# ZhengmaoHe/PARC

Hardware: AMD Instinct MI355X
Metric: env-steps/sec (whole node), 4096 envs/GPU humanoid tracker at 1/2/4/8 MI355X (higher is better)
Workload: dtype f32; 1 GPU; 4096 envs/GPU tracker on procgen box heightfields, 64 synthetic clips (BASELINE.json configs[2]); envs_per_gpu=4096, env_steps_per_bench_step=131072, rollout_steps=32, update_epochs=5, minibatch=16384, sim_substeps=4, parallelism=dp1, scaling_rule=per-rank work fixed (T = 32, minibatch = 4 x envs): weak scaling, grad_allreduce=per minibatch (reference cadence)

## Files before the change

include/parc_hip.h:

```cpp
#ifndef PARC_HIP_H
#define PARC_HIP_H

#include <stdint.h>

#ifdef __cplusplus
extern "C" {
#endif

#define PARC_MAX_BODIES 16
#define PARC_MAX_DOFS 64
#define PARC_MAX_TAR_STEPS 6
#define PARC_MAX_KEY_BODIES 8

#define PARC_OK 0
#define PARC_EINVAL (-1)
#define PARC_EUNSUPPORTED (-2)

#define PARC_JOINT_ROOT 0
#define PARC_JOINT_HINGE 1
#define PARC_JOINT_SPHERICAL 2
#define PARC_JOINT_FIXED 3

#define PARC_DONE_NULL 0
#define PARC_DONE_FAIL 1
#define PARC_DONE_SUCC 2
#define PARC_DONE_TIME 3

typedef struct {
    int32_t num_bodies;
    int32_t dof_size;
    int32_t max_depth;
    int32_t parent[PARC_MAX_BODIES];
    int32_t joint_type[PARC_MAX_BODIES];
    int32_t dof_idx[PARC_MAX_BODIES];
    int32_t depth[PARC_MAX_BODIES];
    float local_translation[PARC_MAX_BODIES][3];
    float local_rotation[PARC_MAX_BODIES][4];
    float joint_axis[PARC_MAX_BODIES][3];
} parc_char_model_t;

typedef struct {
    int32_t num_motions, num_bodies, dof_size, row_stride;
    int32_t off_pos, off_contacts, off_root_vel, off_root_ang_vel, off_dof_vel;
    const int32_t *num_frames;
    const int32_t *start_idx;
    const float *length;
    const int32_t *loop_mode;
    const float *pos_delta;
    const float *frames;
} parc_motion_lib_t;

typedef struct {
    const float *hf;
    int32_t dim_x, dim_y;
    float min_x, min_y, dx, dy;
} parc_terrain_t;

typedef struct {
    int32_t num_tar_steps;
    float tar_dt[PARC_MAX_TAR_STEPS];
    int32_t num_key_bodies;
    int32_t key_body_ids[PARC_MAX_KEY_BODIES];
    float joint_err_w[PARC_MAX_BODIES];
    float dof_err_w[PARC_MAX_DOFS];
    float contact_w[PARC_MAX_BODIES];
    float reward_w[5];
    float rel_deepmimic_w;
    float pose_termination_dist[PARC_MAX_BODIES];
    int32_t pose_termination, enable_early_termination, track_root;
    float root_pos_termination_dist, root_rot_termination_angle, termination_height;
    int32_t num_contact_bodies;
    int32_t contact_body_mask[PARC_MAX_BODIES];
    float episode_length, contact_eps, min_obs_h, max_obs_h;
    int32_t num_ray_points;
    int32_t obs_dim;
    float task1_w, task2_w, target_radius;
    float target_future_min, target_future_max;
    int32_t track_root_h, use_contact_info;
    int32_t global_obs;
} parc_track_cfg_t;

typedef struct {
    int32_t num_envs;
    const float *root_state;
    const float *dof_state;
    const float *rigid_body_state;
    const float *contact_forces;
    const float *env_offsets;
    const int64_t *motion_ids;
    const float *motion_time_offsets;
    const float *motion_xy_offset;
    const float *time_buf;
    const float *target_xy;
    float *ref_root_pos, *ref_root_rot, *ref_root_vel, *ref_root_ang_vel;
    float *ref_joint_rot, *ref_dof_vel, *ref_dof_pos;
    float *ref_contacts, *ref_body_pos;
    float *obs;
    float *reward;
    float *reward_terms;
    int32_t *done;
    int32_t *done_kind;
    const int32_t *env_mask;
    const float *init_noise_xy;
    float *next_target_time;
    const float *target_rand;
    float *obs_aux;
    int32_t reward_terms_stride;
} parc_env_buffers_t;

int parc_refresh_ray_obs_hfs(void *stream, int n_envs, const float *ray_xy, int n_points,
                             const float *root_pos_xyz, const float *heading, parc_terrain_t terrain,
                             float min_h, float max_h, float *out, int64_t out_stride);

int parc_refresh_obs_hfs(void *stream, int n_envs, const float *ray_xy, int n_points, const float *root_state,
                         const float *env_offsets, parc_terrain_t terrain, float min_h, float max_h, float *out,
                         int64_t out_stride);

int parc_dof_to_rot(void *stream, parc_char_model_t model, int n, const float *dof, float *joint_rot);
int parc_rot_to_dof(void *stream, parc_char_model_t model, int n, const float *joint_rot, float *dof);
int parc_forward_kinematics(void *stream, parc_char_model_t model, int n, const float *root_pos, const float *root_rot,
                            const float *joint_rot, float *body_pos, float *body_rot);

int parc_pose_chain_forward(void *stream, parc_char_model_t model, int n, const float *root_pos, const float *root_exp, const float *dof,
                            float *root_quat, float *joint_rot, float *body_pos, float *body_rot);
int parc_pose_chain_backward(void *stream, parc_char_model_t model, int n, const float *root_exp, const float *dof,
                             const float *g_root_quat, const float *g_joint_rot, const float *g_body_pos, const float *g_body_rot,
                             float *g_root_pos, float *g_root_exp, float *g_dof);

int parc_body_points_world(void *stream, int n_frames, int num_bodies, int num_points, const float *body_pos, const float *body_rot,
                           const float *local, const int32_t *owner, float *world);
int parc_body_points_world_grad(void *stream, int n_frames, int num_bodies, int num_points, const float *body_rot, const float *local,
                                const int32_t *start, const float *g_world, float *g_body_pos, float *g_body_rot);

int parc_quat_diff_angle(void *stream, int64_t n, const float *q0, const float *q1, float *angle);
int parc_quat_diff_angle_grad(void *stream, int64_t n, const float *q0, const float *q1, const float *g_angle, float *g_q0, float *g_q1);

int parc_temporal_terms(void *stream, int n_frames, int num_bodies, const float *body_pos, const float *rot_err_sq, const float *src_vel,
                        const float *keep, const float *pair_contact, float c, float c2, float jerk_limit, float *partial);
int parc_temporal_terms_grad(void *stream, int n_frames, int num_bodies, const float *body_pos, const float *rot_err_sq, const float *src_vel,
                             const float *keep, const float *pair_contact, float c, float c2, float jerk_limit, const float *cotangents,
                             float *g_body_pos, float *g_rot_err_sq);

int parc_calc_motion_frame(void *stream, parc_motion_lib_t mlib, int n_queries, const int64_t *motion_ids,
                           const float *motion_times, float *root_pos, float *root_rot, float *root_vel,
                           float *root_ang_vel, float *joint_rot, float *dof_vel, float *contacts);

int parc_motion_lib_build(void *stream, parc_char_model_t model, parc_motion_lib_t mlib, int total_frames,
                          const float *frames, const float *contacts, const int32_t *frame_clip, const float *clip_fps,
                          float *rows);

#define PARC_POST_REF 1
#define PARC_POST_OBS 2
#define PARC_POST_REWARD_DONE 4
#define PARC_POST_HF 8
#define PARC_POST_MASKED 16
#define PARC_POST_INIT_CHAR 32
#define PARC_POST_TARGETS 64
#define PARC_POST_PLAN_CLOCK 128
#define PARC_POST_ALL 255
int parc_track_post_step(void *stream, parc_char_model_t model, parc_motion_lib_t mlib, parc_terrain_t terrain,
                         parc_track_cfg_t cfg, parc_env_buffers_t buf, const int64_t *env_ids, int n_sel, int what,
                         const float *ray_xy);

int parc_track_post_step_timed(void *stream, parc_char_model_t model, parc_motion_lib_t mlib, parc_terrain_t terrain,
                               parc_track_cfg_t cfg, parc_env_buffers_t buf, const int64_t *env_ids, int n_sel, int what,
                               const float *ray_xy, void *start_event, void *stop_event);

int parc_assemble_obs(void *stream, int n_envs, const float *obs, int obs_dim, const float *aux, const float *scalar,
                      const int32_t *col_map, float *out, int out_dim, const int64_t *env_ids, int n_sel);

int parc_reset_apply(void *stream, int n_envs, const int32_t *mask, const int64_t *new_motion_ids, const int64_t *new_terrain_ids,
                     const float *new_time_offsets, const float *motion_offsets, int terrains_per_motion, int64_t *motion_ids,
                     int64_t *motion_terrain_ids, float *motion_time_offsets, float *motion_xy_offset, int32_t *timestep_buf,
                     float *time_buf, int32_t *done, float *next_target_time, int64_t *ep_num);

int parc_reset_sample_apply(void *stream, int n_envs, const int32_t *done_flags, int32_t *mask, const float *uniforms, int n_motions,
                            const float *motion_weights, const float *fail_rates, float min_weight, const float *motion_lengths,
                            const float *motion_offsets, int terrains_per_motion, float noise_scale, float *cdf_workspace,
                            int64_t *motion_ids, int64_t *motion_terrain_ids, float *motion_time_offsets, float *motion_xy_offset,
                            int32_t *timestep_buf, float *time_buf, int32_t *done, float *next_target_time, int64_t *ep_num,
                            float *init_noise_xy);

int parc_step_tail(void *stream, parc_char_model_t model, parc_motion_lib_t mlib, parc_env_buffers_t buf, int what, int n_motions,
                   const int32_t *done_kind, float ema_w, float *fail_rates);
int parc_update_fail_rates(void *stream, int n_envs, int n_motions, const int64_t *motion_ids, const int32_t *done_kind,
                           float ema_w, float *fail_rates);

int parc_td_lambda_return(void *stream, int T, int N, const float *reward, const float *next_vals, const int32_t *done,
                          float discount, float td_lambda, float *ret);
int parc_adv_normalize(void *stream, int n, const float *ret, const float *vals, const float *rand_action_mask,
                       float clip, float *norm_adv, float *mean_std_out , double *workspace);

typedef struct {
    float clip_ratio, bound_w, entropy_w, reg_w, critic_w, large_critic_loss;
    int32_t critic_l1;
} parc_ppo_cfg_t;
int parc_ppo_loss(void *stream, int B, int A, const float *mean, const float *logstd, const float *norm_a, const float *old_logp,
                  const float *adv, const float *mask, const float *pred, const float *tar_val, parc_ppo_cfg_t cfg, float *g_mean,
                  float *g_logstd, float *g_pred, float *out, float *workspace);
int parc_ppo_workspace_floats(int B);
int parc_ppo_loss_packed(void *stream, int B, int A, const float *mean, const float *logstd, const float *rec, int rec_stride,
                         const float *pred, parc_ppo_cfg_t cfg, float *g_mean, float *g_logstd, float *g_pred, float *out,
                         float *workspace);

typedef struct {
    const void *src;
    void *dst;
    int32_t row_bytes;
    int32_t convert;
} parc_record_field_t;
int parc_record_step(void *stream, int n_envs, const int64_t *head, int n_fields, const parc_record_field_t *fields);

int parc_rng_step(void *stream, uint64_t seed, uint64_t *state, float *uniform_out, int64_t n_uniform, float *normal_out, int64_t n_normal,
                  int64_t *tick_cell, int tick_mod);

int64_t parc_sgd_workspace_floats(void);
int parc_sgd_momentum_step(void *stream, int64_t n, float *params, const float *grad, float *momentum_buf, float max_norm, float lr,
                           float momentum, float weight_decay, float *workspace, float *norm_out);

int parc_adamw_step(void *stream, int64_t n, float *params, const float *grad, float *exp_avg, float *exp_avg_sq, int64_t step,
                    float max_norm, float lr, float beta1, float beta2, float eps, float weight_decay, float *workspace, float *norm_out);

int parc_normalize_clamp(void *stream, int64_t rows, int dim, const float *x, const float *mean, const float *stdv, float clip, float *out);

int64_t parc_moments_workspace_floats(int64_t rows, int dim);
int parc_moments_accumulate(void *stream, int64_t rows, int dim, const float *x, float *acc, float *workspace);
int parc_obs_ingest(void *stream, int64_t rows, int dim, const float *x, const float *mean, const float *stdv, float clip, float *norm_out,
                    float *copy_dst, const int64_t *copy_row, float *acc, float *workspace);

int parc_action_head(void *stream, int n, int A, const float *mean, const float *logstd, const float *noise, const float *explore,
                     const float *a_mean, const float *a_std, float *action, float *logp);
int parc_action_head_record(void *stream, int n, int A, const float *mean, const float *logstd, const float *noise, const float *explore,
                            const float *a_mean, const float *a_std, float *action, float *logp, float *rec_action, float *rec_logp,
                            float *rec_mask, const float *forces_src, float *rec_forces, int n_forces, const int64_t *head);

int parc_points_hf_sdf(void *stream, int batch, int n_points, int dim_x, int dim_y, const float *points, const float *hf,
                       const float *min_box_center, const float *x_points, const float *y_points, float half_x, float half_y,
                       float base_z, int inverted, float radius, float *out, int32_t *out_cell);

int parc_points_hf_sdf_grad(void *stream, int batch, int n_points, int dim_x, int dim_y, const float *points, const float *hf,
                            const float *min_box_center, const float *x_points, const float *y_points, float half_x, float half_y,
                            float base_z, int inverted, const int32_t *cell, const float *g_out, float *g_points);

int64_t parc_relu_bwd_workspace_floats(int64_t rows, int dim);
int parc_relu_bwd_bias_grad(void *stream, int64_t rows, int dim, float *gy, const float *y, float *db, float *workspace);
int parc_weighted_colsum(void *stream, int64_t rows, int dim, const float *x, const float *w, float *out, float *workspace);

int parc_abi_version(void);

#ifdef __cplusplus
}
#endif
#endif
```

parc_amd/_hip.py:

```python
import ctypes
import os
import subprocess

import torch

_HERE = os.path.dirname(os.path.abspath(__file__))
LIB_DIR = os.path.join(_HERE, "lib")
LIB_PATH = os.path.join(LIB_DIR, "libparc_hip.so")
CSRC = os.path.join(_HERE, "csrc")
SOURCES = ["parc_kin.hip", "parc_sim.hip", "parc_ppo.hip", "parc_rollout.hip", "parc_optim.hip", "parc_colreduce.hip", "parc_terrain.hip", "parc_render.hip", "parc_score.hip", "parc_netstats.hip", "parc_moopt.hip",
           "parc_augment.hip", "parc_mdm_batch.hip", "parc_mdm_loss.hip", "parc_mdm_guide.hip", "parc_mdm_gen.hip", "parc_hfgather.hip", "parc_motion.hip", "parc_pose_opt.hip", "parc_returns.hip"]
DIAG_LIB_PATH = os.path.join(LIB_DIR, "libparc_hip_diag.so")
DIAG_SOURCES = SOURCES + ["parc_sim_ref.hip"]

MAX_BODIES = 16
MAX_DOFS = 64
MAX_TAR_STEPS = 6
MAX_KEY_BODIES = 8

POST_REF = 1
POST_OBS = 2
POST_REWARD_DONE = 4
POST_HF = 8
POST_MASKED = 16
POST_INIT_CHAR = 32
POST_TARGETS = 64
POST_PLAN_CLOCK = 128

c_int = ctypes.c_int
c_i32 = ctypes.c_int32
c_i64 = ctypes.c_int64
c_f = ctypes.c_float
c_vp = ctypes.c_void_p


class CharModelS(ctypes.Structure):
    _fields_ = [("num_bodies", c_i32), ("dof_size", c_i32), ("max_depth", c_i32),
                ("parent", c_i32 * MAX_BODIES), ("joint_type", c_i32 * MAX_BODIES), ("dof_idx", c_i32 * MAX_BODIES),
                ("depth", c_i32 * MAX_BODIES),
                ("local_translation", (c_f * 3) * MAX_BODIES), ("local_rotation", (c_f * 4) * MAX_BODIES),
                ("joint_axis", (c_f * 3) * MAX_BODIES)]


class MotionLibS(ctypes.Structure):
    _fields_ = [("num_motions", c_i32), ("num_bodies", c_i32), ("dof_size", c_i32), ("row_stride", c_i32),
                ("off_pos", c_i32), ("off_contacts", c_i32), ("off_root_vel", c_i32), ("off_root_ang_vel", c_i32),
                ("off_dof_vel", c_i32),
                ("num_frames", c_vp), ("start_idx", c_vp), ("length", c_vp), ("loop_mode", c_vp), ("pos_delta", c_vp),
                ("frames", c_vp)]


class TerrainS(ctypes.Structure):
    _fields_ = [("hf", c_vp), ("dim_x", c_i32), ("dim_y", c_i32), ("min_x", c_f), ("min_y", c_f), ("dx", c_f), ("dy", c_f)]


class TrackCfgS(ctypes.Structure):
    _fields_ = [("num_tar_steps", c_i32), ("tar_dt", c_f * MAX_TAR_STEPS),
                ("num_key_bodies", c_i32), ("key_body_ids", c_i32 * MAX_KEY_BODIES),
                ("joint_err_w", c_f * MAX_BODIES), ("dof_err_w", c_f * MAX_DOFS), ("contact_w", c_f * MAX_BODIES),
                ("reward_w", c_f * 5), ("rel_deepmimic_w", c_f),
                ("pose_termination_dist", c_f * MAX_BODIES),
                ("pose_termination", c_i32), ("enable_early_termination", c_i32), ("track_root", c_i32),
                ("root_pos_termination_dist", c_f), ("root_rot_termination_angle", c_f), ("termination_height", c_f),
                ("num_contact_bodies", c_i32), ("contact_body_mask", c_i32 * MAX_BODIES),
                ("episode_length", c_f), ("contact_eps", c_f), ("min_obs_h", c_f), ("max_obs_h", c_f),
                ("num_ray_points", c_i32), ("obs_dim", c_i32),
                ("task1_w", c_f), ("task2_w", c_f), ("target_radius", c_f),
                ("target_future_min", c_f), ("target_future_max", c_f), ("track_root_h", c_i32), ("use_contact_info", c_i32), ("global_obs", c_i32)]


class EnvBuffersS(ctypes.Structure):
    _fields_ = [("num_envs", c_i32),
                ("root_state", c_vp), ("dof_state", c_vp), ("rigid_body_state", c_vp), ("contact_forces", c_vp),
                ("env_offsets", c_vp), ("motion_ids", c_vp), ("motion_time_offsets", c_vp), ("motion_xy_offset", c_vp),
                ("time_buf", c_vp), ("target_xy", c_vp),
                ("ref_root_pos", c_vp), ("ref_root_rot", c_vp), ("ref_root_vel", c_vp), ("ref_root_ang_vel", c_vp),
                ("ref_joint_rot", c_vp), ("ref_dof_vel", c_vp), ("ref_dof_pos", c_vp),
                ("ref_contacts", c_vp), ("ref_body_pos", c_vp),
                ("obs", c_vp), ("reward", c_vp), ("reward_terms", c_vp), ("done", c_vp), ("done_kind", c_vp),
                ("env_mask", c_vp), ("init_noise_xy", c_vp), ("next_target_time", c_vp), ("target_rand", c_vp), ("obs_aux", c_vp),
                ("reward_terms_stride", c_i32)]


class RecordFieldS(ctypes.Structure):
    _fields_ = [("src", c_vp), ("dst", c_vp), ("row_bytes", c_i32), ("convert", c_i32)]


class PPOCfgS(ctypes.Structure):
    _fields_ = [("clip_ratio", c_f), ("bound_w", c_f), ("entropy_w", c_f), ("reg_w", c_f), ("critic_w", c_f),
                ("large_critic_loss", c_f), ("critic_l1", c_i32)]


_lib = None


NO_SLP = "-O3 -fno-slp-vectorize"
OPT_LEVEL = {"parc_kin.hip": os.environ.get("PARC_KIN_OPT", NO_SLP), "parc_sim.hip": os.environ.get("PARC_SIM_OPT", NO_SLP), "parc_sim_ref.hip": "-O2",
             "parc_hfgather.hip": NO_SLP, "parc_motion.hip": NO_SLP, "parc_pose_opt.hip": NO_SLP, "parc_returns.hip": NO_SLP,
             "parc_augment.hip": "-O3 -ffp-contract=off",
             "parc_mdm_batch.hip": "-O3 -ffp-contract=off",
             "parc_mdm_loss.hip": "-O3 -ffp-contract=off",
             "parc_mdm_guide.hip": "-O3 -ffp-contract=off",
             "parc_mdm_gen.hip": "-O3 -ffp-contract=off"}


DIGEST_PATH = os.path.join(LIB_DIR, "libparc_hip.digest")
DIAG_DIGEST_PATH = os.path.join(LIB_DIR, "libparc_hip_diag.digest")


def source_digest():
    import hashlib
    h = hashlib.sha256()
    inc = os.path.join(os.path.dirname(_HERE), "include")
    files = [os.path.join(CSRC, f) for f in sorted(os.listdir(CSRC)) if f.endswith((".hip", ".h"))] + \
        ([os.path.join(inc, f) for f in sorted(os.listdir(inc)) if f.endswith(".h")] if os.path.isdir(inc) else [])
    for f in files:
        h.update(os.path.basename(f).encode())
        with open(f, "rb") as fh:
            h.update(fh.read())
    h.update(repr((DIAG_SOURCES, sorted(OPT_LEVEL.items()))).encode())
    return h.hexdigest()


def _stored_digest(path=DIGEST_PATH):
    try:
        with open(path) as f:
            return f.read().strip()
    except OSError:
        return None


def build(force=False, verbose=False, diag=False):
    lib_path, digest_path, sources = (DIAG_LIB_PATH, DIAG_DIGEST_PATH, DIAG_SOURCES) if diag else (LIB_PATH, DIGEST_PATH, SOURCES)
    digest = source_digest()
    if not force and os.path.exists(lib_path) and _stored_digest(digest_path) == digest:
        return lib_path
    obj_dir = os.path.join(LIB_DIR, "obj_diag" if diag else "obj")
    os.makedirs(obj_dir, exist_ok=True)
    hipcc = os.environ.get("HIPCC", "/opt/rocm/bin/hipcc")
    objs, procs = [], []
    for s in sources:
        o = os.path.join(obj_dir, s.replace(".hip", ".o"))
        cmd = [hipcc, "--offload-arch=gfx950"] + OPT_LEVEL.get(s, "-O3").split() + (["-DPARC_DIAG_BUILD"] if diag else []) + \
            ["-std=c++17", "-fPIC", "-c", "-o", o, os.path.join(CSRC, s)]
        if verbose:
            print(" ".join(cmd))
        procs.append((cmd, subprocess.Popen(cmd)))
        objs.append(o)
    for cmd, p in procs:
        if p.wait() != 0:
            raise subprocess.CalledProcessError(p.returncode, cmd)
    cmd = [hipcc, "--offload-arch=gfx950", "-shared", "-fPIC", "-o", lib_path] + objs
    if verbose:
        print(" ".join(cmd))
    subprocess.check_call(cmd)
    with open(digest_path, "w") as f:
        f.write(digest + "\n")
    return lib_path


def lib():
    global _lib
    if _lib is None:
        if not os.path.exists(LIB_PATH):
            raise RuntimeError("libparc_hip.so is not built ({}); run `python -c 'import __graft_entry__ as g; g.build()'` "
                               "-- there is no CPU fallback".format(LIB_PATH))
        if _stored_digest() != source_digest():
            raise RuntimeError("libparc_hip.so was built from other sources than the ones beside it (csrc/, include/): rebuild with "
                               "`python -c 'import __graft_entry__ as g; g.build()'` - calling a stale library would hand it argument "
                               "structs of another layout")
        _lib = ctypes.CDLL(LIB_PATH)
        _declare(_lib)
    return _lib


def _declare(L):
    L.parc_abi_version.restype = c_int
    L.parc_refresh_ray_obs_hfs.argtypes = [c_vp, c_int, c_vp, c_int, c_vp, c_vp, TerrainS, c_f, c_f, c_vp, c_i64]
    L.parc_refresh_obs_hfs.argtypes = [c_vp, c_int, c_vp, c_int, c_vp, c_vp, TerrainS, c_f, c_f, c_vp, c_i64]
    L.parc_dof_to_rot.argtypes = [c_vp, CharModelS, c_int, c_vp, c_vp]
    L.parc_rot_to_dof.argtypes = [c_vp, CharModelS, c_int, c_vp, c_vp]
    L.parc_forward_kinematics.argtypes = [c_vp, CharModelS, c_int, c_vp, c_vp, c_vp, c_vp, c_vp]
    L.parc_pose_chain_forward.argtypes = [c_vp, CharModelS, c_int, c_vp, c_vp, c_vp, c_vp, c_vp, c_vp, c_vp]
    L.parc_pose_chain_backward.argtypes = [c_vp, CharModelS, c_int, c_vp, c_vp, c_vp, c_vp, c_vp, c_vp, c_vp, c_vp, c_vp]
    L.parc_body_points_world.argtypes = [c_vp, c_int, c_int, c_int, c_vp, c_vp, c_vp, c_vp, c_vp]
    L.parc_body_points_world_grad.argtypes = [c_vp, c_int, c_int, c_int, c_vp, c_vp, c_vp, c_vp, c_vp, c_vp]
    L.parc_quat_diff_angle.argtypes = [c_vp, ctypes.c_int64, c_vp, c_vp, c_vp]
    L.parc_quat_diff_angle_grad.argtypes = [c_vp, ctypes.c_int64, c_vp, c_vp, c_vp, c_vp, c_vp]
    L.parc_temporal_terms.argtypes = [c_vp, c_int, c_int, c_vp, c_vp, c_vp, c_vp, c_vp, c_f, c_f, c_f, c_vp]
    L.parc_temporal_terms_grad.argtypes = [c_vp, c_int, c_int, c_vp, c_vp, c_vp, c_vp, c_vp, c_f, c_f, c_f, c_vp, c_vp, c_vp]
    L.parc_calc_motion_frame.argtypes = [c_vp, MotionLibS, c_int, c_vp, c_vp] + [c_vp] * 7
    L.parc_motion_lib_build.argtypes = [c_vp, CharModelS, MotionLibS, c_int, c_vp, c_vp, c_vp, c_vp, c_vp]
    L.parc_track_post_step.argtypes = [c_vp, CharModelS, MotionLibS, TerrainS, TrackCfgS, EnvBuffersS, c_vp, c_int, c_int, c_vp]
    L.parc_track_post_step_timed.argtypes = L.parc_track_post_step.argtypes + [c_vp, c_vp]
    L.parc_track_post_step_timed.restype = c_int
    L.parc_assemble_obs.argtypes = [c_vp, c_int, c_vp, c_int, c_vp, c_vp, c_vp, c_vp, c_int, c_vp, c_int]
    L.parc_assemble_obs.restype = c_int
    L.parc_update_fail_rates.argtypes = [c_vp, c_int, c_int, c_vp, c_vp, c_f, c_vp]
    L.parc_step_tail.argtypes = [c_vp, CharModelS, MotionLibS, EnvBuffersS, c_int, c_int, c_vp, c_f, c_vp]
    L.parc_step_tail.restype = c_int
    L.parc_td_lambda_return.argtypes = [c_vp, c_int, c_int, c_vp, c_vp, c_vp, c_f, c_f, c_vp]
    L.parc_adv_normalize.argtypes = [c_vp, c_int, c_vp, c_vp, c_vp, c_f, c_vp, c_vp, c_vp]
    L.parc_ppo_loss.argtypes = [c_vp, c_int, c_int] + [c_vp] * 8 + [PPOCfgS] + [c_vp] * 5
    L.parc_ppo_loss.restype = c_int
    L.parc_ppo_loss_packed.argtypes = [c_vp, c_int, c_int, c_vp, c_vp, c_vp, c_int, c_vp, PPOCfgS] + [c_vp] * 5
    L.parc_ppo_loss_packed.restype = c_int
    L.parc_ppo_workspace_floats.argtypes = [c_int]
    L.parc_ppo_workspace_floats.restype = c_int
    L.parc_normalize_clamp.argtypes = [c_vp, c_i64, c_int, c_vp, c_vp, c_vp, c_f, c_vp]
    L.parc_normalize_clamp.restype = c_int
    L.parc_action_head.argtypes = [c_vp, c_int, c_int] + [c_vp] * 8
    L.parc_action_head.restype = c_int
    L.parc_action_head_record.argtypes = [c_vp, c_int, c_int] + [c_vp] * 8 + [c_vp] * 5 + [c_int, c_vp]
    L.parc_action_head_record.restype = c_int
    L.parc_points_hf_sdf.argtypes = [c_vp, c_int, c_int, c_int, c_int] + [c_vp] * 5 + [c_f, c_f, c_f, c_int, c_f, c_vp, c_vp]
    L.parc_points_hf_sdf.restype = c_int
    L.parc_points_hf_sdf_grad.argtypes = [c_vp, c_int, c_int, c_int, c_int] + [c_vp] * 5 + [c_f, c_f, c_f, c_int, c_vp, c_vp, c_vp]
    L.parc_points_hf_sdf_grad.restype = c_int
    L.parc_scale_by_clipped_norm.argtypes = [c_vp, c_i64, c_vp, c_vp, c_f]
    L.parc_scale_by_clipped_norm.restype = c_int
    L.parc_moments_workspace_floats.argtypes = [c_i64, c_int]
    L.parc_moments_workspace_floats.restype = c_i64
    L.parc_moments_accumulate.argtypes = [c_vp, c_i64, c_int, c_vp, c_vp, c_vp]
    L.parc_moments_accumulate.restype = c_int
    L.parc_relu_bwd_workspace_floats.argtypes = [c_i64, c_int]
    L.parc_relu_bwd_workspace_floats.restype = c_i64
    L.parc_relu_bwd_bias_grad.argtypes = [c_vp, c_i64, c_int, c_vp, c_vp, c_vp, c_vp]
    L.parc_relu_bwd_bias_grad.restype = c_int
    L.parc_weighted_colsum.argtypes = [c_vp, c_i64, c_int, c_vp, c_vp, c_vp, c_vp]
    L.parc_weighted_colsum.restype = c_int
    L.parc_sgd_workspace_floats.argtypes = []
    L.parc_sgd_workspace_floats.restype = c_i64
    L.parc_sgd_momentum_step.argtypes = [c_vp, c_i64, c_vp, c_vp, c_vp, c_f, c_f, c_f, c_f, c_vp, c_vp]
    L.parc_sgd_momentum_step.restype = c_int
    L.parc_adamw_step.argtypes = [c_vp, c_i64, c_vp, c_vp, c_vp, c_vp, c_i64, c_f, c_f, c_f, c_f, c_f, c_f, c_vp, c_vp]
    L.parc_adamw_step.restype = c_int
    L.parc_return_tracker_update.argtypes = [c_vp, c_int, c_int, c_vp, c_i64] + [c_vp] * 8
    L.parc_return_tracker_workspace_floats.argtypes = [c_int]
    L.parc_return_tracker_workspace_floats.restype = c_i64
    L.parc_return_tracker_update.restype = c_int
    L.parc_record_step.argtypes = [c_vp, c_int, c_vp, c_int, c_vp]
    L.parc_record_step.restype = c_int
    L.parc_obs_ingest.argtypes = [c_vp, c_i64, c_int, c_vp, c_vp, c_vp, c_f, c_vp, c_vp, c_vp, c_vp, c_vp]
    L.parc_obs_ingest.restype = c_int
    L.parc_rng_step.argtypes = [c_vp, ctypes.c_uint64, c_vp, c_vp, c_i64, c_vp, c_i64, c_vp, c_int]
    L.parc_rng_step.restype = c_int
    L.parc_reset_apply.argtypes = [c_vp, c_int, c_vp, c_vp, c_vp, c_vp, c_vp, c_int] + [c_vp] * 9
    L.parc_reset_apply.restype = c_int
    L.parc_reset_sample_apply.argtypes = [c_vp, c_int, c_vp, c_vp, c_vp, c_int, c_vp, c_vp, c_f, c_vp, c_vp, c_int, c_f] + [c_vp] * 11
    L.parc_reset_sample_apply.restype = c_int
    for name in ("parc_refresh_ray_obs_hfs", "parc_refresh_obs_hfs", "parc_dof_to_rot", "parc_rot_to_dof",
                 "parc_forward_kinematics", "parc_calc_motion_frame", "parc_motion_lib_build", "parc_track_post_step", "parc_reset_apply",
                 "parc_update_fail_rates", "parc_td_lambda_return", "parc_adv_normalize"):
        getattr(L, name).restype = c_int
    if hasattr(L, "parc_sim_abi"):
        from . import _hip_sim
        _hip_sim.declare(L)
    if hasattr(L, "parc_render_abi"):
        from . import _hip_render
        _hip_render.declare(L)
    if hasattr(L, "parc_score_abi"):
        from . import _hip_score
        _hip_score.declare(L)
    if hasattr(L, "parc_netstats_abi"):
        from . import _hip_netstats
        _hip_netstats.declare(L)
    if hasattr(L, "parc_moopt_abi"):
        from . import _hip_moopt
        _hip_moopt.declare(L)
    if hasattr(L, "parc_augment_abi"):
        from . import _hip_augment
        _hip_augment.declare(L)
    if hasattr(L, "parc_mdm_batch_abi"):
        from . import _hip_mdm_batch
        _hip_mdm_batch.declare(L)
    if hasattr(L, "parc_mdm_loss_abi"):
        from . import _hip_mdm_loss
        _hip_mdm_loss.declare(L)
    if hasattr(L, "parc_mdm_guide_abi"):
        from . import _hip_mdm_guide
        _hip_mdm_guide.declare(L)
    if hasattr(L, "parc_mdm_gen_abi"):
        from . import _hip_mdm_gen
        _hip_mdm_gen.declare(L)


EXPORTED = ["parc_abi_version", "parc_refresh_ray_obs_hfs", "parc_refresh_obs_hfs", "parc_dof_to_rot", "parc_rot_to_dof",
            "parc_forward_kinematics", "parc_calc_motion_frame", "parc_motion_lib_build", "parc_track_post_step",
            "parc_update_fail_rates", "parc_td_lambda_return", "parc_adv_normalize", "parc_reset_apply", "parc_ppo_loss", "parc_ppo_workspace_floats", "parc_record_step", "parc_return_tracker_update", "parc_normalize_clamp",
            "parc_action_head", "parc_points_hf_sdf", "parc_moments_workspace_floats", "parc_moments_accumulate", "parc_reset_sample_apply", "parc_return_tracker_workspace_floats", "parc_scale_by_clipped_norm", "parc_relu_bwd_workspace_floats",
            "parc_relu_bwd_bias_grad", "parc_ppo_loss_packed", "parc_weighted_colsum", "parc_sgd_workspace_floats", "parc_sgd_momentum_step", "parc_adamw_step",
            "parc_pose_chain_forward", "parc_pose_chain_backward", "parc_points_hf_sdf_grad", "parc_body_points_world", "parc_body_points_world_grad",
            "parc_quat_diff_angle", "parc_quat_diff_angle_grad", "parc_temporal_terms", "parc_temporal_terms_grad", "parc_step_tail",
            "parc_assemble_obs", "parc_track_post_step_timed", "parc_rng_step", "parc_obs_ingest", "parc_action_head_record",
            "parc_render", "parc_render_abi", "parc_motion_score", "parc_score_abi",
            "parc_netstats_workspace_floats", "parc_netstats_update", "parc_netstats_abs_colsum", "parc_netstats_dormant_count", "parc_netstats_abi",
            "parc_points_hf_sdf_ragged", "parc_points_hf_sdf_ragged_grad", "parc_temporal_terms_seg", "parc_temporal_terms_seg_grad",
            "parc_segment_sums", "parc_moopt_abi",
            "parc_augment_frames", "parc_augment_terrains", "parc_augment_localize", "parc_augment_abi",
            "parc_mdm_heightfields", "parc_mdm_windows", "parc_mdm_batch_abi",
            "parc_mdm_loss_forward", "parc_mdm_loss_backward", "parc_mdm_loss_lds_bytes", "parc_mdm_loss_abi",
            "parc_mdm_guide_step", "parc_mdm_guide_lds_bytes", "parc_mdm_guide_abi",
            "parc_mdm_gen_encode", "parc_mdm_gen_decode", "parc_mdm_gen_abi"]


def check(rc, what):
    if rc != 0:
        raise RuntimeError("{} failed with code {} ({})".format(what, rc, "bad argument" if rc == -1 else "unsupported" if rc == -2 else "hipError"))


def stream():
    return c_vp(torch.cuda.current_stream().cuda_stream)


def ptr(t):
    if t is None:
        return c_vp(0)
    assert t.is_cuda, "HIP kernels need device tensors (no CPU fallback)"
    assert t.is_contiguous(), "tensor must be contiguous"
    return c_vp(t.data_ptr())


def terrain_struct(hf, min_point, dxdy):
    assert hf.dtype == torch.float32 and hf.is_contiguous() and hf.dim() == 2
    return TerrainS(ptr(hf), int(hf.shape[0]), int(hf.shape[1]), float(min_point[0]), float(min_point[1]),
                    float(dxdy[0]), float(dxdy[1]))


class HipEventPair:
    _rt = None

    def __init__(self):
        if HipEventPair._rt is None:
            HipEventPair._rt = ctypes.CDLL("libamdhip64.so")
        self.start, self.stop = c_vp(), c_vp()
        for ev in (self.start, self.stop):
            rc = HipEventPair._rt.hipEventCreate(ctypes.byref(ev))
            if rc != 0:
                raise RuntimeError("hipEventCreate -> %d" % rc)

    def elapsed_us(self):
        ms = ctypes.c_float()
        rc = HipEventPair._rt.hipEventElapsedTime(ctypes.byref(ms), self.start, self.stop)
        if rc != 0:
            raise RuntimeError("hipEventElapsedTime -> %d" % rc)
        return ms.value * 1e3

    def __del__(self):
        try:
            for ev in (self.start, self.stop):
                if ev:
                    HipEventPair._rt.hipEventDestroy(ev)
        except Exception:
            pass
```

parc_amd/csrc/parc_colreduce.hip:

```cpp
#include <hip/hip_runtime.h>
#include <stdint.h>

#include "../../include/parc_hip.h"
#include "parc_launch.h"
#include "parc_learner_math.h"

__global__ __launch_bounds__(256) void normalize_clamp_kernel(size_t n4, int dim4, const float4 *__restrict__ x, const float4 *__restrict__ mean,
                                                              const float4 *__restrict__ stdv, float clip, float4 *__restrict__ out) {
    for (size_t i = (size_t)blockIdx.x * blockDim.x + threadIdx.x; i < n4; i += (size_t)gridDim.x * blockDim.x) {
        const int c = (int)(i % (size_t)dim4);
        const float4 v = x[i], m = mean[c], s = stdv[c];
        float4 o;
        o.x = clamp_nan((v.x - m.x) / s.x, -clip, clip);
        o.y = clamp_nan((v.y - m.y) / s.y, -clip, clip);
        o.z = clamp_nan((v.z - m.z) / s.z, -clip, clip);
        o.w = clamp_nan((v.w - m.w) / s.w, -clip, clip);
        out[i] = o;
    }
}

extern "C" int parc_normalize_clamp(void *stream, int64_t rows, int dim, const float *x, const float *mean, const float *stdv, float clip,
                                    float *out) {
    if (rows < 0 || dim <= 0 || (dim & 3) || (((uintptr_t)x | (uintptr_t)mean | (uintptr_t)stdv | (uintptr_t)out) & 15)) return PARC_EINVAL;
    if (rows == 0) return PARC_OK;
    const size_t n4 = (size_t)rows * (size_t)(dim / 4);
    hipLaunchKernelGGL(normalize_clamp_kernel, dim3(parc_capped_blocks(n4, 8192)), dim3(256), 0, (hipStream_t)stream, n4, dim / 4, (const float4 *)x,
                       (const float4 *)mean, (const float4 *)stdv, clip, (float4 *)out);
    PARC_CHECK_LAUNCH();
    return PARC_OK;
}

struct col_chunk_t {
    int lane, rg, c, r0, r1;
};

__device__ __forceinline__ col_chunk_t col_chunk(int rows, int chunk_rows) {
    const int lane = threadIdx.x & 63, r0 = blockIdx.y * chunk_rows;
    return {lane, (int)(threadIdx.x >> 6), (int)(blockIdx.x * 64 + lane), r0, min(r0 + chunk_rows, rows)};
}

__device__ __forceinline__ float4 fold_row_groups(const float4 (*red)[64], int lane) {
    const float4 a = red[0][lane], b = red[1][lane], d = red[2][lane], e = red[3][lane];
    float4 o;
    o.x = (a.x + b.x) + (d.x + e.x); o.y = (a.y + b.y) + (d.y + e.y); o.z = (a.z + b.z) + (d.z + e.z); o.w = (a.w + b.w) + (d.w + e.w);
    return o;
}

__device__ __forceinline__ void fold_store(float4 (*red)[64], const float4 &s, const col_chunk_t &k, int dim4, float4 *__restrict__ partial) {
    red[k.rg][k.lane] = s;
    __syncthreads();
    if (k.rg == 0 && k.c < dim4) partial[(size_t)blockIdx.y * dim4 + k.c] = fold_row_groups(red, k.lane);
}

__device__ __forceinline__ void fold_store_moments(float4 (*red)[4][64], const float4 &s, const float4 &q, const col_chunk_t &k, int dim4,
                                                   float4 *__restrict__ partial) {
    red[0][k.rg][k.lane] = s;
    red[1][k.rg][k.lane] = q;
    __syncthreads();
    if (k.rg < 2 && k.c < dim4) partial[((size_t)blockIdx.y * 2 + k.rg) * dim4 + k.c] = fold_row_groups(red[k.rg], k.lane);
}

struct col_grid_t {
    int rc, dim4, chunks;
    dim3 grid;
};

static col_grid_t col_chunk_grid(int64_t rows, int dim, int chunk_rows, uintptr_t aligned16, bool missing) {
    if (rows < 0 || dim <= 0 || (dim & 3) || missing || (aligned16 & 15)) return {PARC_EINVAL};
    if (rows > (int64_t)chunk_rows * 65535) return {PARC_EUNSUPPORTED};
    const int dim4 = dim / 4, chunks = (int)((rows + chunk_rows - 1) / chunk_rows);
    return {PARC_OK, dim4, chunks, dim3((dim4 + 63) / 64, chunks)};
}

#define MOM_ROWS 64
__global__ __launch_bounds__(256) void moments_partial_kernel(int rows, int dim4, const float4 *__restrict__ x, float4 *__restrict__ partial) {
    __shared__ float4 red[2][4][64];
    const col_chunk_t k = col_chunk(rows, MOM_ROWS);
    const int rg = k.rg, c = k.c, r0 = k.r0, r1 = k.r1;
    float4 s = make_float4(0.f, 0.f, 0.f, 0.f), q = s;
    if (c < dim4) {
        for (int r = r0 + rg; r < r1; r += 4) {
            const float4 v = x[(size_t)r * dim4 + c];
            s.x += v.x; s.y += v.y; s.z += v.z; s.w += v.w;
            q.x = fmaf(v.x, v.x, q.x); q.y = fmaf(v.y, v.y, q.y); q.z = fmaf(v.z, v.z, q.z); q.w = fmaf(v.w, v.w, q.w);
        }
    }
    fold_store_moments(red, s, q, k, dim4, partial);
}

__global__ __launch_bounds__(256) void obs_ingest_kernel(int rows, int dim4, const float4 *__restrict__ x, const float4 *__restrict__ mean,
                                                         const float4 *__restrict__ stdv, float clip, float4 *__restrict__ norm_out,
                                                         float4 *copy_dst, const int64_t *__restrict__ copy_row, float4 *partial) {
    __shared__ float4 red[2][4][64];
    const col_chunk_t k = col_chunk(rows, MOM_ROWS);
    const int rg = k.rg, c = k.c, r0 = k.r0, r1 = k.r1;
    float4 s = make_float4(0.f, 0.f, 0.f, 0.f), q = s;
    if (c < dim4) {
        const float4 m = mean[c], sd = stdv[c];
        float4 *dst = copy_dst ? copy_dst + (size_t)copy_row[0] * (size_t)rows * dim4 : nullptr;
        for (int r = r0 + rg; r < r1; r += 4) {
            const size_t i = (size_t)r * dim4 + c;
            const float4 v = x[i];
            float4 o;
            o.x = clamp_nan((v.x - m.x) / sd.x, -clip, clip);
            o.y = clamp_nan((v.y - m.y) / sd.y, -clip, clip);
            o.z = clamp_nan((v.z - m.z) / sd.z, -clip, clip);
            o.w = clamp_nan((v.w - m.w) / sd.w, -clip, clip);
            norm_out[i] = o;
            if (dst) {
                typedef float f32x4 __attribute__((ext_vector_type(4)));
                f32x4 vv = {v.x, v.y, v.z, v.w};
                __builtin_nontemporal_store(vv, reinterpret_cast<f32x4 *>(dst) + i);
            }
            s.x += v.x; s.y += v.y; s.z += v.z; s.w += v.w;
            q.x = fmaf(v.x, v.x, q.x); q.y = fmaf(v.y, v.y, q.y); q.z = fmaf(v.z, v.z, q.z); q.w = fmaf(v.w, v.w, q.w);
        }
    }
    if (!partial) return;
    fold_store_moments(red, s, q, k, dim4, partial);
}

__global__ __launch_bounds__(256) void moments_final_kernel(int chunks, int dim4, const float4 *__restrict__ partial, float4 *acc) {
    const int i = blockIdx.x * blockDim.x + threadIdx.x;
    if (i >= 2 * dim4) return;
    const int which = i / dim4, c = i - which * dim4;
    float4 t = make_float4(0.f, 0.f, 0.f, 0.f);
#pragma unroll 16
    for (int k = 0; k < chunks; ++k) {
        const float4 v = partial[((size_t)k * 2 + which) * dim4 + c];
        t.x += v.x; t.y += v.y; t.z += v.z; t.w += v.w;
    }
    float4 a = acc[i];
    a.x += t.x; a.y += t.y; a.z += t.z; a.w += t.w;
    acc[i] = a;
}

static void launch_moments_final(void *stream, const col_grid_t &g, const float *workspace, float *acc) {
    hipLaunchKernelGGL(moments_final_kernel, dim3((2 * g.dim4 + 255) / 256), dim3(256), 0, (hipStream_t)stream, g.chunks, g.dim4,
                       (const float4 *)workspace, (float4 *)acc);
}

extern "C" int64_t parc_moments_workspace_floats(int64_t rows, int dim) {
    if (rows < 0 || dim <= 0) return -1;
    return ((rows + MOM_ROWS - 1) / MOM_ROWS) * 2 * (int64_t)dim;
}

extern "C" int parc_obs_ingest(void *stream, int64_t rows, int dim, const float *x, const float *mean, const float *stdv, float clip, float *norm_out,
                               float *copy_dst, const int64_t *copy_row, float *acc, float *workspace) {
    const col_grid_t g = col_chunk_grid(rows, dim, MOM_ROWS,
                                        (uintptr_t)x | (uintptr_t)mean | (uintptr_t)stdv | (uintptr_t)norm_out | (uintptr_t)copy_dst | (uintptr_t)acc | (uintptr_t)workspace,
                                        !x || !mean || !stdv || !norm_out || (copy_dst && !copy_row) || (acc && !workspace));
    if (g.rc != PARC_OK || rows == 0) return g.rc;
    hipLaunchKernelGGL(obs_ingest_kernel, g.grid, dim3(256), 0, (hipStream_t)stream, (int)rows, g.dim4, (const float4 *)x, (const float4 *)mean,
                       (const float4 *)stdv, clip, (float4 *)norm_out, (float4 *)copy_dst, copy_row, acc ? (float4 *)workspace : (float4 *)nullptr);
    if (acc) launch_moments_final(stream, g, workspace, acc);
    PARC_CHECK_LAUNCH();
    return PARC_OK;
}

extern "C" int parc_moments_accumulate(void *stream, int64_t rows, int dim, const float *x, float *acc, float *workspace) {
    const col_grid_t g = col_chunk_grid(rows, dim, MOM_ROWS, (uintptr_t)x | (uintptr_t)acc | (uintptr_t)workspace, false);
    if (g.rc != PARC_OK || rows == 0) return g.rc;
    hipLaunchKernelGGL(moments_partial_kernel, g.grid, dim3(256), 0, (hipStream_t)stream, (int)rows, g.dim4, (const float4 *)x, (float4 *)workspace);
    launch_moments_final(stream, g, workspace, acc);
    PARC_CHECK_LAUNCH();
    return PARC_OK;
}

#define RB_ROWS 128
__global__ __launch_bounds__(256) void relu_bwd_bias_partial_kernel(int rows, int dim4, float4 *__restrict__ gy, const float4 *__restrict__ y,
                                                                    float4 *__restrict__ partial) {
    __shared__ float4 red[4][64];
    const col_chunk_t k = col_chunk(rows, RB_ROWS);
    const int rg = k.rg, c = k.c, r0 = k.r0, r1 = k.r1;
    float4 s = make_float4(0.f, 0.f, 0.f, 0.f);
    if (c < dim4) {
#pragma unroll 4
        for (int r = r0 + rg; r < r1; r += 4) {
            const size_t i = (size_t)r * dim4 + c;
            float4 g = gy[i];
            const float4 a = y[i];
            g.x = a.x <= 0.f ? 0.f : g.x; g.y = a.y <= 0.f ? 0.f : g.y; g.z = a.z <= 0.f ? 0.f : g.z; g.w = a.w <= 0.f ? 0.f : g.w;
            gy[i] = g;
            s.x += g.x; s.y += g.y; s.z += g.z; s.w += g.w;
        }
    }
    fold_store(red, s, k, dim4, partial);
}

__global__ __launch_bounds__(256) void colsum_final_kernel(int chunks, int dim, const float *__restrict__ partial, float *__restrict__ out) {
    const int c = blockIdx.x * blockDim.x + threadIdx.x;
    if (c >= dim) return;
    float t = 0.f;
#pragma unroll 16
    for (int k = 0; k < chunks; ++k) t += partial[(size_t)k * dim + c];
    out[c] = t;
}

__global__ __launch_bounds__(256) void weighted_colsum_partial_kernel(int rows, int dim4, const float4 *__restrict__ x, const float *__restrict__ w,
                                                                      float4 *__restrict__ partial) {
    __shared__ float4 red[4][64];
    const col_chunk_t k = col_chunk(rows, RB_ROWS);
    const int rg = k.rg, c = k.c, r0 = k.r0, r1 = k.r1;
    float4 s = make_float4(0.f, 0.f, 0.f, 0.f);
    if (c < dim4) {
#pragma unroll 4
        for (int r = r0 + rg; r < r1; r += 4) {
            const float4 v = x[(size_t)r * dim4 + c];
            const float wr = w[r];
            s.x = fmaf(wr, v.x, s.x); s.y = fmaf(wr, v.y, s.y); s.z = fmaf(wr, v.z, s.z); s.w = fmaf(wr, v.w, s.w);
        }
    }
    fold_store(red, s, k, dim4, partial);
}

static void launch_colsum_final(void *stream, const col_grid_t &g, int dim, const float *workspace, float *out) {
    hipLaunchKernelGGL(colsum_final_kernel, dim3((dim + 255) / 256), dim3(256), 0, (hipStream_t)stream, g.chunks, dim, workspace, out);
}

extern "C" int parc_weighted_colsum(void *stream, int64_t rows, int dim, const float *x, const float *w, float *out, float *workspace) {
    const col_grid_t g = col_chunk_grid(rows, dim, RB_ROWS, (uintptr_t)x | (uintptr_t)workspace, !x || !w || !out || !workspace);
    if (g.rc != PARC_OK) return g.rc;
    if (rows > 0)
        hipLaunchKernelGGL(weighted_colsum_partial_kernel, g.grid, dim3(256), 0, (hipStream_t)stream, (int)rows, g.dim4, (const float4 *)x, w,
                           (float4 *)workspace);
    launch_colsum_final(stream, g, dim, workspace, out);
    PARC_CHECK_LAUNCH();
    return PARC_OK;
}

extern "C" int64_t parc_relu_bwd_workspace_floats(int64_t rows, int dim) {
    if (rows < 0 || dim <= 0) return -1;
    return ((rows + RB_ROWS - 1) / RB_ROWS) * (int64_t)dim;
}

extern "C" int parc_relu_bwd_bias_grad(void *stream, int64_t rows, int dim, float *gy, const float *y, float *db, float *workspace) {
    const col_grid_t g = col_chunk_grid(rows, dim, RB_ROWS, (uintptr_t)gy | (uintptr_t)y | (uintptr_t)workspace, !gy || !y || !db || !workspace);
    if (g.rc != PARC_OK) return g.rc;
    if (rows > 0)
        hipLaunchKernelGGL(relu_bwd_bias_partial_kernel, g.grid, dim3(256), 0, (hipStream_t)stream, (int)rows, g.dim4, (float4 *)gy, (const float4 *)y,
                           (float4 *)workspace);
    launch_colsum_final(stream, g, dim, workspace, db);
    PARC_CHECK_LAUNCH();
    return PARC_OK;
}
```

parc_amd/csrc/parc_ppo.hip:

```cpp
#include <hip/hip_runtime.h>

#include "../../include/parc_hip.h"
#include "parc_launch.h"
#include "parc_learner_math.h"

#define PPO_THREADS 256
#define PPO_MAX_A 64
#define PPO_NSCAL 8
#define PPO_W (PPO_NSCAL + PPO_MAX_A)

struct ppo_surr_t {
    float ratio, surr, c;
};

__device__ __forceinline__ ppo_surr_t ppo_surrogate(int A, float zz, float sum_logstd, const float *old_logp, const float *adv, size_t si, bool sel,
                                                    float m, parc_ppo_cfg_t cfg) {
    ppo_surr_t s;
    const float logp = -0.5f * zz + (-0.5f * (float)A * 1.8378770664093453f - sum_logstd);
    s.ratio = __expf(logp - old_logp[si]);
    const float ad = adv[si];
    const float lo = 1.0f - cfg.clip_ratio, hi = 1.0f + cfg.clip_ratio;
    const float rc = clamp_nan(s.ratio, lo, hi);
    const float l0 = ad * s.ratio, l1 = ad * rc;
    s.surr = minimum_nan(l0, l1);
    const float dsurr = (l0 <= l1) ? ad : ((s.ratio >= lo && s.ratio <= hi) ? ad : 0.f);
    s.c = sel ? -m * dsurr * s.ratio : 0.f;
    return s;
}

__device__ __forceinline__ float ppo_critic_grad(parc_ppo_cfg_t cfg, float diff) {
    return cfg.critic_l1 ? (diff > 0.f ? -1.f : (diff < 0.f ? 1.f : 0.f)) : -2.0f * diff;
}

__global__ __launch_bounds__(PPO_THREADS) void ppo_sample_kernel(int B, int A, const float *__restrict__ mean, const float *__restrict__ logstd,
                                                                 const float *__restrict__ norm_a, const float *__restrict__ old_logp,
                                                                 const float *__restrict__ adv, const float *__restrict__ mask,
                                                                 const float *__restrict__ pred, const float *__restrict__ tar_val,
                                                                 parc_ppo_cfg_t cfg, float *g_mean, float *g_pred, float *ws, int a_stride,
                                                                 int s_stride) {
    __shared__ float s_istd[PPO_MAX_A];
    __shared__ float s_part[PPO_THREADS / 64][PPO_W];
    const int tid = threadIdx.x, i = blockIdx.x * PPO_THREADS + tid;
    float sum_logstd = 0.f;
    if (tid < A) s_istd[tid] = __expf(-logstd[tid]);
    __syncthreads();
    for (int j = 0; j < A; ++j) sum_logstd += logstd[j];
    const bool live = i < B;
    const int ii = live ? i : 0;
    const size_t si = (size_t)ii * s_stride;
    const bool sel = live && mask[si] == 1.0f;
    const float m = sel ? 1.f : 0.f;
    const float *mu = mean + (size_t)ii * A, *ac = norm_a + (size_t)ii * a_stride;
    float zz = 0.f, viol = 0.f, reg = 0.f;
    for (int j = 0; j < A; ++j) {
        float mj = mu[j];
        float z = (ac[j] - mj) * s_istd[j];
        zz = fmaf(z, z, zz);
        float vmin = clamp_max_nan(mj + 1.0f, 0.f), vmax = clamp_min_nan(mj - 1.0f, 0.f);
        viol += vmin * vmin + vmax * vmax;
        reg = fmaf(mj, mj, reg);
    }
    const ppo_surr_t sr = ppo_surrogate(A, zz, sum_logstd, old_logp, adv, si, sel, m, cfg);
    const float c = sr.c;
    const float diff = tar_val[si] - pred[ii];
    if (live) {
        g_pred[i] = ppo_critic_grad(cfg, diff);
        float *gm = g_mean + (size_t)i * A;
        for (int j = 0; j < A; ++j) {
            float mj = mu[j];
            float z = (ac[j] - mj) * s_istd[j];
            float vmin = clamp_max_nan(mj + 1.0f, 0.f), vmax = clamp_min_nan(mj - 1.0f, 0.f);
            gm[j] = sel ? c * z * s_istd[j] + m * (cfg.bound_w * 2.0f * (vmin + vmax) + cfg.reg_w * 2.0f * mj) : 0.f;
        }
    }
    float sc[PPO_NSCAL];
    sc[0] = m;
    sc[1] = live ? (cfg.critic_l1 ? fabsf(diff) : diff * diff) : 0.f;
    sc[2] = sel ? m * sr.surr : 0.f;
    sc[3] = m * (fabsf(sr.ratio - 1.0f) > cfg.clip_ratio ? 1.f : 0.f);
    sc[4] = sel ? m * sr.ratio : 0.f;
    sc[5] = sel ? m * viol : 0.f;
    sc[6] = sel ? m * reg : 0.f;
    sc[7] = 0.f;
    const int wv = tid >> 6, ln = tid & 63;
#pragma unroll
    for (int k = 0; k < PPO_NSCAL; ++k) {
        float v = wave_sum(sc[k]);
        if (ln == 0) s_part[wv][k] = v;
    }
    for (int j = 0; j < A; ++j) {
        float z = live ? (ac[j] - mu[j]) * s_istd[j] : 0.f;
        float v = wave_sum(sel ? c * (z * z - 1.0f) : 0.f);
        if (ln == 0) s_part[wv][PPO_NSCAL + j] = v;
    }
    __syncthreads();
    if (tid < PPO_NSCAL + A) {
        float v = 0.f;
#pragma unroll
        for (int w = 0; w < PPO_THREADS / 64; ++w) v += s_part[w][tid];
        ws[(size_t)blockIdx.x * PPO_W + tid] = v;
    }
}

#define PPO32_SPB 64
__global__ __launch_bounds__(256) void ppo_sample32_kernel(int B, int A, const float *__restrict__ mean, const float *__restrict__ logstd,
                                                           const float *__restrict__ norm_a, const float *__restrict__ old_logp,
                                                           const float *__restrict__ adv, const float *__restrict__ mask,
                                                           const float *__restrict__ pred, const float *__restrict__ tar_val, parc_ppo_cfg_t cfg,
                                                           float *g_mean, float *g_pred, float *ws, int a_stride, int s_stride) {
    __shared__ float s_part[8][PPO_W];
    const int tid = threadIdx.x, g = tid >> 5, j = tid & 31;
    const bool vj = j < A;
    const float ls = vj ? logstd[j] : 0.f;
    const float istd = __expf(-ls);
    float sum_logstd = ls;
#pragma unroll
    for (int o = 16; o >= 1; o >>= 1) sum_logstd += __shfl_xor(sum_logstd, o, 32);
    float acc[PPO_NSCAL];
#pragma unroll
    for (int k = 0; k < PPO_NSCAL; ++k) acc[k] = 0.f;
    float acc_ls = 0.f;
#pragma unroll 2
    for (int it = 0; it < PPO32_SPB / 8; ++it) {
        const int i = blockIdx.x * PPO32_SPB + it * 8 + g;
        const bool live = i < B;
        const int ii = live ? i : 0;
        const size_t si = (size_t)ii * s_stride;
        const bool sel = live && mask[si] == 1.0f;
        const float m = sel ? 1.f : 0.f;
        const float mj = vj ? mean[(size_t)ii * A + j] : 0.f;
        const float aj = vj ? norm_a[(size_t)ii * a_stride + j] : 0.f;
        const float z = (aj - mj) * istd;
        const float vmin = clamp_max_nan(mj + 1.0f, 0.f), vmax = clamp_min_nan(mj - 1.0f, 0.f);
        float zz = vj ? z * z : 0.f, viol = vj ? vmin * vmin + vmax * vmax : 0.f, reg = vj ? mj * mj : 0.f;
#pragma unroll
        for (int o = 16; o >= 1; o >>= 1) {
            zz += __shfl_xor(zz, o, 32);
            viol += __shfl_xor(viol, o, 32);
            reg += __shfl_xor(reg, o, 32);
        }
        const ppo_surr_t sr = ppo_surrogate(A, zz, sum_logstd, old_logp, adv, si, sel, m, cfg);
        const float c = sr.c;
        const float diff = tar_val[si] - pred[ii];
        if (live) {
            if (j == 0) g_pred[i] = ppo_critic_grad(cfg, diff);
            if (vj) g_mean[(size_t)i * A + j] = sel ? c * z * istd + m * (cfg.bound_w * 2.0f * (vmin + vmax) + cfg.reg_w * 2.0f * mj) : 0.f;
        }
        acc[0] += m;
        acc[1] += live ? (cfg.critic_l1 ? fabsf(diff) : diff * diff) : 0.f;
        acc[2] += sel ? m * sr.surr : 0.f;
        acc[3] += m * (fabsf(sr.ratio - 1.0f) > cfg.clip_ratio ? 1.f : 0.f);
        acc[4] += sel ? m * sr.ratio : 0.f;
        acc[5] += sel ? m * viol : 0.f;
        acc[6] += sel ? m * reg : 0.f;
        acc_ls += (sel && vj) ? c * (z * z - 1.0f) : 0.f;
    }
    if (j == 0) {
#pragma unroll
        for (int k = 0; k < PPO_NSCAL; ++k) s_part[g][k] = acc[k];
    }
    if (vj) s_part[g][PPO_NSCAL + j] = acc_ls;
    __syncthreads();
    if (tid < PPO_NSCAL + A) {
        float v = 0.f;
#pragma unroll
        for (int w = 0; w < 8; ++w) v += s_part[w][tid];
        ws[(size_t)blockIdx.x * PPO_W + tid] = v;
    }
}

#define PPO_RED_THREADS (4 * PPO_W)
__global__ __launch_bounds__(PPO_RED_THREADS) void ppo_reduce_kernel(int B, int A, int nblk, const float *__restrict__ logstd, parc_ppo_cfg_t cfg,
                                                                    const float *__restrict__ ws, float *g_logstd, float *out) {
    __shared__ float s[PPO_W];
    __shared__ double s4[PPO_W][4];
    const int tid = threadIdx.x;
    {
        const int v = tid >> 2, part = tid & 3;
        const int per = (nblk + 3) >> 2, b0 = part * per, b1 = min(b0 + per, nblk);
        double acc = 0.0;
        if (v < PPO_NSCAL + A) {
#pragma unroll 16
            for (int b = b0; b < b1; ++b) acc += (double)ws[(size_t)b * PPO_W + v];
        }
        s4[v][part] = acc;
    }
    __syncthreads();
    if (tid < PPO_NSCAL + A) s[tid] = (float)((s4[tid][0] + s4[tid][1]) + (s4[tid][2] + s4[tid][3]));
    __syncthreads();
    const float msum = s[0];
    const float cnt = msum;
    const float critic_loss = s[1] / (float)B;
    float sum_logstd = 0.f;
    for (int j = 0; j < A; ++j) sum_logstd += logstd[j];
    const float ent = (sum_logstd + 0.5f * (float)A * 2.8378770664093453f) * (msum / cnt);
    const float abl = s[5] / cnt, regl = s[6] / cnt;
    float actor_loss = -s[2] / cnt;
    if (cfg.bound_w != 0.f) actor_loss += cfg.bound_w * abl;
    if (cfg.entropy_w != 0.f) actor_loss -= cfg.entropy_w * ent;
    if (cfg.reg_w != 0.f) actor_loss += cfg.reg_w * regl;
    const float gate = critic_loss > cfg.large_critic_loss ? 0.f : 1.f;
    if (tid < A) g_logstd[tid] = gate * (s[PPO_NSCAL + tid] / cnt - cfg.entropy_w * (msum / cnt));
    if (tid == 0) {
        out[0] = actor_loss + cfg.critic_w * critic_loss;
        out[1] = critic_loss;
        out[2] = actor_loss;
        out[3] = s[3] / cnt;
        out[4] = s[4] / cnt;
        out[5] = abl;
        out[6] = ent;
        out[7] = regl;
        out[8] = cnt;
        out[9] = gate / cnt;
        out[10] = cfg.critic_w / (float)B;
    }
}

__global__ __launch_bounds__(256) void ppo_scale_kernel(int n_mean, int n_pred, const float *__restrict__ out, float *g_mean, float *g_pred) {
    const int i = blockIdx.x * blockDim.x + threadIdx.x;
    const float sa = out[9], sp = out[10];
    if (i < n_mean) g_mean[i] *= sa;
    if (i < n_pred) g_pred[i] *= sp;
}

static int ppo_loss_impl(void *stream, int B, int A, const float *mean, const float *logstd, const float *norm_a, const float *old_logp,
                         const float *adv, const float *mask, const float *pred, const float *tar_val, parc_ppo_cfg_t cfg, float *g_mean,
                         float *g_logstd, float *g_pred, float *out, float *workspace, int a_stride, int s_stride) {
    if (B <= 0 || A <= 0 || A > PPO_MAX_A) return PARC_EINVAL;
    int nblk = (B + PPO_THREADS - 1) / PPO_THREADS;
    hipStream_t st = (hipStream_t)stream;
    if (A <= 32) {
        nblk = (B + PPO32_SPB - 1) / PPO32_SPB;
        hipLaunchKernelGGL(ppo_sample32_kernel, dim3(nblk), dim3(256), 0, st, B, A, mean, logstd, norm_a, old_logp, adv, mask, pred, tar_val, cfg,
                           g_mean, g_pred, workspace, a_stride, s_stride);
    } else {
        hipLaunchKernelGGL(ppo_sample_kernel, dim3(nblk), dim3(PPO_THREADS), 0, st, B, A, mean, logstd, norm_a, old_logp, adv, mask, pred, tar_val,
                           cfg, g_mean, g_pred, workspace, a_stride, s_stride);
    }
    hipLaunchKernelGGL(ppo_reduce_kernel, dim3(1), dim3(PPO_RED_THREADS), 0, st, B, A, nblk, logstd, cfg, workspace, g_logstd, out);
    const int n = B * A;
    hipLaunchKernelGGL(ppo_scale_kernel, dim3((n + 255) / 256), dim3(256), 0, st, n, B, out, g_mean, g_pred);
    PARC_CHECK_LAUNCH();
    return PARC_OK;
}

extern "C" int parc_ppo_loss(void *stream, int B, int A, const float *mean, const float *logstd, const float *norm_a, const float *old_logp,
                             const float *adv, const float *mask, const float *pred, const float *tar_val, parc_ppo_cfg_t cfg, float *g_mean,
                             float *g_logstd, float *g_pred, float *out, float *workspace) {
    return ppo_loss_impl(stream, B, A, mean, logstd, norm_a, old_logp, adv, mask, pred, tar_val, cfg, g_mean, g_logstd, g_pred, out, workspace, A, 1);
}

extern "C" int parc_ppo_loss_packed(void *stream, int B, int A, const float *mean, const float *logstd, const float *rec, int rec_stride,
                                    const float *pred, parc_ppo_cfg_t cfg, float *g_mean, float *g_logstd, float *g_pred, float *out,
                                    float *workspace) {
    if (!rec || rec_stride < A + 4) return PARC_EINVAL;
    return ppo_loss_impl(stream, B, A, mean, logstd, rec, rec + A, rec + A + 1, rec + A + 2, pred, rec + A + 3, cfg, g_mean, g_logstd, g_pred, out,
                         workspace, rec_stride, rec_stride);
}

extern "C" int parc_ppo_workspace_floats(int B) { return ((B + PPO32_SPB - 1) / PPO32_SPB) * PPO_W; }
```

parc_amd/learning/dm_ppo_agent.py:

```python
import enum
import os
import time

import numpy as np
import torch

from ..envs import base_env
from ..gym_spaces import Box
from ..util import mp_util
from ..util.logger import Logger
from . import dm_ppo_model, experience_buffer, mp_optimizer, normalizer, rl_util, unit_stats
from .dm_ppo_return_tracker import DMPPOReturnTracker
from .tracking_error_tracker import TrackingErrorTracker


class AgentMode(enum.Enum):
    TRAIN = 0
    TEST = 1


_LOSS_KEYS = ["norm_obs", "action", "a_logp", "tar_val", "adv", "rand_action_mask"]


def enable_tuned_gemms():
    import torch.cuda.tunable as tunable
    path = os.path.join(os.path.dirname(os.path.dirname(os.path.abspath(__file__))), "tunableop_results.csv")
    if not os.path.exists(path) or tunable.is_enabled():
        return
    tunable.set_filename(path, False)
    tunable.tuning_enable(False)
    if hasattr(tunable, "write_file_on_exit"):
        tunable.write_file_on_exit(False)
    tunable.enable(True)


class DMPPOAgent(torch.nn.Module):
    NAME = "DM_PPO"

    def __init__(self, config, env, device):
        super().__init__()
        self._env = env
        self._device = device
        self._iter = 0
        self._sample_count = 0
        self._config = config
        self._is_terrain_runner = env.NAME in ("ig_terrain_runner", "ig_parkour")
        self._has_target_task = env.NAME in ("ig_terrain_runner", "ig_deepmimic_terrain", "ig_parkour")
        self._load_params(config)
        self._build_normalizers()
        self._model = dm_ppo_model.DMPPOModel(config["model"], env)
        self.to(self._device)
        params = [p for p in self.parameters() if p.requires_grad]
        self._optimizer = mp_optimizer.MPOptimizer(config["optimizer"], params)
        self._build_exp_buffer(config)
        self._train_return_tracker = DMPPOReturnTracker(self.get_num_envs(), self._device, self._has_target_task)
        self._test_return_tracker = DMPPOReturnTracker(self.get_num_envs(), self._device, self._has_target_task)
        self._mode = AgentMode.TRAIN
        self._curr_obs = None
        self._curr_info = None
        self._ppo_cfg = None
        if str(self._device).startswith("cuda") and config.get("tuned_gemms", True):
            enable_tuned_gemms()
        self._use_hip_graph = bool(config.get("hip_graph_rollout", True)) and str(self._device).startswith("cuda")
        self._graphs = dict()
        self._graph_pool = None
        self._graph_warm = 0
        self._exp_prob_t = torch.ones([1, 1], dtype=torch.float32, device=self._device)
        self._head_t = torch.zeros([1], dtype=torch.int64, device=self._device)
        self._head_dev, self._exp_prob_dev = 0, 1.0
        self._compute_times = []
        self._replan_time_rows, self._replan_time_src = None, None
        self._ones_mask = None
        self._unit_stats = None
        self._unit_report = None
        if getattr(self._env, "_report_tracking_error", False):
            self._test_tracking_error_tracker = TrackingErrorTracker(self.get_num_envs(), self._device)

    @staticmethod
    def rollout_shape(config, num_procs):
        P = int(num_procs) if config.get("mp_scale_rollout", True) else 1
        return int(np.ceil(config["steps_per_iter"] / P)), int(np.ceil(config["batch_size"] / P))

    def _load_params(self, config):
        self._discount = config["discount"]
        self._iters_per_output = config["iters_per_output"]
        self._iters_per_checkpoint = config["iters_per_checkpoint"]
        self._normalizer_samples = config.get("normalizer_samples", np.inf)
        self._test_episodes = config["test_episodes"]
        self._steps_per_iter, self._batch_size = self.rollout_shape(config, mp_util.get_num_procs())
        self._update_epochs = config["update_epochs"]
        self._td_lambda = config["td_lambda"]
        self._ppo_clip_ratio = config["ppo_clip_ratio"]
        self._norm_adv_clip = config["norm_adv_clip"]
        self._action_bound_weight = config["action_bound_weight"]
        self._action_entropy_weight = config["action_entropy_weight"]
        self._action_reg_weight = config["action_reg_weight"]
        self._critic_loss_weight = config["critic_loss_weight"]
        self._exp_anneal_samples = config.get("exp_anneal_samples", np.inf)
        self._exp_prob_beg = config.get("exp_prob_beg", 1.0)
        self._exp_prob_end = config.get("exp_prob_end", 1.0)
        self._clip_grad_norm = config.get("clip_grad_norm", False)
        self._max_grad_norm = config.get("max_grad_norm", 0.5)
        self._critic_loss_type = config.get("critic_loss_type", "L2")
        self._log_unit_stats = bool(config.get("log_unit_stats", False))

    def _build_normalizers(self):
        obs_space = self._env.get_obs_space()
        shapes = self._env._compute_obs(ret_obs_shapes=True)
        idx, cur = [], 0
        for key in shapes:
            shape = shapes[key]["shape"]
            flat = shape[0] * shape[1] if len(shape) >= 2 else shape[0]
            if not shapes[key]["use_normalizer"]:
                idx.append(torch.arange(cur, cur + flat, dtype=torch.int64, device=self._device))
            cur += flat
        non_norm = torch.cat(idx) if idx else None
        self._obs_norm = normalizer.Normalizer(obs_space.shape, device=self._device, dtype=torch.float32, non_norm_indices=non_norm,
                                               clip=self._config["norm_obs_clip"])
        a_space = self._env.get_action_space()
        assert isinstance(a_space, Box)
        a_mean = torch.tensor(0.5 * (a_space.high + a_space.low), device=self._device, dtype=torch.float32)
        a_std = torch.tensor(0.5 * (a_space.high - a_space.low), device=self._device, dtype=torch.float32)
        self._a_norm = normalizer.Normalizer(a_mean.shape, device=self._device, init_mean=a_mean, init_std=a_std, dtype=torch.float32)

    def _build_exp_buffer(self, config):
        T, N, dev = self._steps_per_iter, self.get_num_envs(), self._device
        self._exp_buffer = experience_buffer.ExperienceBuffer(buffer_length=T, batch_size=N, device=dev)
        obs_dim = list(self._env.get_obs_space().shape)
        a_dim = list(self._env.get_action_space().shape)
        B = self._env._cfg.num_bodies if hasattr(self._env, "_cfg") else 15

        def add(name, shape, dtype=torch.float32):
            self._exp_buffer.add_buffer(name, torch.zeros([T, N] + shape, device=dev, dtype=dtype))
        add("obs", obs_dim)
        add("next_obs", obs_dim)
        add("action", a_dim)
        add("reward", [])
        add("done", [], torch.int)
        add("a_logp", [])
        add("tar_val", [])
        add("adv", [])
        add("rand_action_mask", [])
        add("timestep", [], torch.int)
        add("ep_num", [], torch.int)
        add("compute_time", [])
        add("prev_char_contact_forces", [B, 3])
        add("next_char_contact_forces", [B, 3])
        add("env_id", [], torch.int64)
        add("norm_obs", obs_dim)
        self._loss_rec_w = ((a_dim[0] if isinstance(a_dim, (list, tuple)) else int(a_dim)) + 4 + 3) // 4 * 4
        add("loss_rec", [self._loss_rec_w])
        self._env_ids = torch.arange(0, N, 1, device=dev, dtype=torch.int64)
        if self._is_terrain_runner:
            add("replan_timer", [])
            add("replan_counter", [], torch.int64)

    def get_num_envs(self):
        return self._env.get_num_envs()

    def get_action_size(self):
        return int(np.prod(self._env.get_action_space().shape))

    def calc_num_params(self):
        return sum(p.numel() for p in self.parameters() if p.requires_grad)

    def set_mode(self, mode):
        self._mode = mode
        self._env.set_mode(base_env.EnvMode.TRAIN if mode == AgentMode.TRAIN else base_env.EnvMode.TEST)

    def save(self, out_file):
        if mp_util.is_root_proc():
            torch.save(self.state_dict(), out_file)

    def load(self, in_file):
        self.load_state_dict(torch.load(in_file, map_location=self._device, weights_only=True))
        self._optimizer.sync()
        Logger.print("Loaded model parameters from {:s}".format(in_file))

    def _get_exp_prob(self):
        if np.isfinite(self._exp_anneal_samples):
            l = float(np.clip(float(self._sample_count) / self._exp_anneal_samples, 0.0, 1.0))
            return (1.0 - l) * self._exp_prob_beg + l * self._exp_prob_end
        return self._exp_prob_beg

    def _set_exp_prob(self, exp_prob):
        if not getattr(self, "_in_graph_step", False):
            self._exp_prob_t.fill_(exp_prob)
            self._exp_prob_dev = exp_prob

    def _need_normalizer_update(self):
        return self._sample_count < self._normalizer_samples

    @torch.no_grad()
    def _decide_action(self, obs, info):
        self._obs_ingested = self._action_recorded = False
        if getattr(self, "_in_graph_step", False) and self._mode == AgentMode.TRAIN and self._obs_norm.can_ingest(obs) \
                and obs.shape[0] == self.get_num_envs() and self._exp_buffer._device_head is not None:
            norm_obs = self._obs_norm.ingest(obs, record=self._need_normalizer_update(),
                                             copy_into=(self._exp_buffer.get_data("obs"), self._exp_buffer._device_head))
            self._obs_ingested = True
        else:
            norm_obs = self._obs_norm.normalize(obs)
        dist = self._model.eval_actor(norm_obs) if self._unit_stats is None else self._eval_actor_with_unit_stats(norm_obs)
        if obs.is_cuda and dist.logstd.dim() == 2 and dist.logstd.stride(0) == 0 and self._config.get("fused_action_head", True):
            return self._decide_action_fused(dist, obs.shape[0])
        if self._mode == AgentMode.TRAIN:
            exp_prob = self._get_exp_prob()
            if exp_prob >= 1.0:
                norm_a = dist.sample()
                mask = torch.ones_like(norm_a[..., 0])
            else:
                self._set_exp_prob(exp_prob)
                mask = torch.bernoulli(self._exp_prob_t.expand(obs.shape[0], 1))
                norm_a = torch.where(mask == 1.0, dist.sample(), dist.mode)
                mask = mask.squeeze(-1)
        else:
            norm_a = dist.mode
            mask = torch.zeros_like(norm_a[..., 0])
        logp = dist.log_prob(norm_a)
        a = self._a_norm.unnormalize(norm_a)
        return a, {"a_logp": logp, "rand_action_mask": mask}

    def _decide_action_fused(self, dist, n):
        from .. import _hip
        mean = dist.mean.contiguous()
        A = mean.shape[1]
        if self._mode == AgentMode.TRAIN:
            exp_prob = self._get_exp_prob()
            if exp_prob >= 1.0:
                if self._ones_mask is None or self._ones_mask.shape[0] != n:
                    self._ones_mask = torch.ones(n, dtype=torch.float32, device=mean.device)
                mask = self._ones_mask
            else:
                self._set_exp_prob(exp_prob)
                mask = torch.bernoulli(self._exp_prob_t.expand(n, 1)).squeeze(-1).contiguous()
            noise = self._step_noise if (getattr(self, "_step_noise", None) is not None and self._step_noise.shape == mean.shape) else torch.randn_like(mean)
        else:
            mask = torch.zeros(n, dtype=torch.float32, device=mean.device)
            noise = mean
        a = torch.empty_like(mean)
        logp = torch.empty(n, dtype=torch.float32, device=mean.device)
        p = _hip.ptr
        eb = self._exp_buffer
        self._action_recorded = False
        if (getattr(self, "_in_graph_step", False) and self._mode == AgentMode.TRAIN and A <= 32 and eb._device_head is not None and n == self.get_num_envs()
                and hasattr(self._env, "_char_contact_forces")):
            f = self._env._char_contact_forces
            nf = f[0].numel()
            _hip.check(_hip.lib().parc_action_head_record(_hip.stream(), n, A, p(mean), p(dist.logstd[0].contiguous()), p(noise), p(mask),
                                                          p(self._a_norm.get_mean()), p(self._a_norm.get_std()), p(a), p(logp),
                                                          p(eb.get_data("action")), p(eb.get_data("a_logp")), p(eb.get_data("rand_action_mask")),
                                                          p(f.contiguous()), p(eb.get_data("prev_char_contact_forces")), nf, p(eb._device_head)),
                       "parc_action_head_record")
            self._action_recorded = True
            return a, {"a_logp": logp, "rand_action_mask": mask}
        _hip.check(_hip.lib().parc_action_head(_hip.stream(), n, A, p(mean), p(dist.logstd[0].contiguous()), p(noise), p(mask),
                                               p(self._a_norm.get_mean()), p(self._a_norm.get_std()), p(a), p(logp)), "parc_action_head")
        return a, {"a_logp": logp, "rand_action_mask": mask}

    def _eval_actor_with_unit_stats(self, norm_obs):
        st = self._unit_stats
        dist, acts = self._model.eval_actor_tapped(norm_obs)
        st.update(acts, dist.mean)
        if st.print_every and st.steps % st.print_every == 0:
            Logger.print("\n".join(unit_stats.report_lines(st.report())))
        return dist

    def _unit_stats_on(self, print_every=0):
        self._unit_stats = unit_stats.UnitStats(self._model, self.get_num_envs(), self._device, tap=getattr(self, "_unit_stats_tap", None))
        self._unit_stats.print_every = int(print_every)

    def _unit_stats_off(self, ranks=None):
        st, self._unit_stats = self._unit_stats, None
        if st is not None:
            self._unit_report = dict(st.report())
            if ranks is not None:
                self._unit_report = {"ranks": ranks, **self._unit_report}

    def unit_report(self):
        return self._unit_report

    def test_model2(self, num_episodes, verbose=False, k=100):
        unit_stats.check_model(self._model)
        self.eval()
        self.set_mode(AgentMode.TEST)
        ranks = unit_stats.model_rank_figures(self._model)
        Logger.print("\n".join(unit_stats.rank_lines(ranks)))
        self._curr_obs, self._curr_info = self._env.reset()
        self._unit_stats_on(print_every=k if verbose else 0)
        try:
            info = self._rollout_test(int(np.ceil(num_episodes / mp_util.get_num_procs())))
            self._unit_stats_off(ranks)
        finally:
            self._unit_stats = None
        Logger.print("\n".join(unit_stats.report_lines(self._unit_report)))
        return info

    def step(self):
        action, action_info = self._decide_action(self._curr_obs, self._curr_info)
        next_obs, r, done, next_info = self._env.step(action)
        return next_obs, r, done, next_info, action, action_info

    def _record_data_pre_step(self, obs, info, action, action_info):
        eb = self._exp_buffer
        if getattr(self, "_in_graph_step", False):
            ingested = getattr(self, "_obs_ingested", False)
            if self._need_normalizer_update() and not ingested:
                self._obs_norm.record(obs)
            items = [] if ingested else [("obs", obs)]
            if not getattr(self, "_action_recorded", False):
                items += [("action", action), ("a_logp", action_info["a_logp"]), ("rand_action_mask", action_info["rand_action_mask"]),
                          ("prev_char_contact_forces", self._env._char_contact_forces)]
            if items:
                eb.record_group(items)
            return
        eb.record("obs", obs)
        eb.record("action", action)
        if self._need_normalizer_update():
            self._obs_norm.record(obs)
        eb.record("a_logp", action_info["a_logp"])
        eb.record("rand_action_mask", action_info["rand_action_mask"])
        eb.record("prev_char_contact_forces", self._env._char_contact_forces if getattr(self, "_in_graph_step", False)
                  else info["char_contact_forces"])

    def _record_data_post_step(self, next_obs, r, done, next_info):
        eb = self._exp_buffer
        if getattr(self, "_in_graph_step", False):
            items = [("next_obs", next_obs), ("reward", r), ("done", done), ("timestep", next_info["timestep"]),
                     ("ep_num", next_info["ep_num"]), ("next_char_contact_forces", next_info["char_contact_forces"]),
                     ("env_id", self._env_ids)]
            if self._is_terrain_runner:
                items += [("replan_timer", self._env.get_replan_time_buf()), ("replan_counter", self._env.get_replan_counter())]
            eb.record_group(items)
            return
        eb.record("next_obs", next_obs)
        eb.record("reward", r)
        eb.record("done", done)
        eb.record("timestep", next_info["timestep"])
        eb.record("ep_num", next_info["ep_num"])
        if not getattr(self, "_in_graph_step", False):
            eb.get_data("compute_time")[eb._buffer_head].fill_(float(next_info["compute_time"]))
        eb.record("next_char_contact_forces", next_info["char_contact_forces"])
        eb.record("env_id", self._env_ids)
        if self._is_terrain_runner:
            eb.record("replan_timer", self._env.get_replan_time_buf().expand(self.get_num_envs()))
            eb.record("replan_counter", self._env.get_replan_counter())

    def _reset_done_envs(self, done):
        done_indices = (done != base_env.DoneFlags.NULL.value).nonzero(as_tuple=False).flatten()
        return self._env.reset(done_indices)

    def _device_tick(self):
        return hasattr(self._env, "step_randoms") and self._config.get("device_step_randoms", True)

    def _train_step_body(self, device_reset=False):
        self._step_noise = None
        if getattr(self, "_in_graph_step", False) and self._device_tick():
            self._step_noise = self._env.step_randoms(self.get_action_size(), tick=(self._head_t, self._exp_buffer._buffer_length))
        action, action_info = self._decide_action(self._curr_obs, self._curr_info)
        self._record_data_pre_step(self._curr_obs, self._curr_info, action, action_info)
        next_obs, r, done, next_info = self._env.step(action)
        self._train_return_tracker.update(next_info, done)
        self._record_data_post_step(next_obs, r, done, next_info)
        if device_reset:
            self._curr_obs, self._curr_info = self._env.reset_done(done)
        return done

    def _device_reset_ok(self):
        env = self._env
        return self._graph_ok() and hasattr(env, "reset_done") and env.supports_device_reset()

    def _graph_ok(self):
        env = self._env
        return (self._use_hip_graph and self._mode == AgentMode.TRAIN and not getattr(env, "_write_agent_states_flag", False)
                and hasattr(env, "_char_contact_forces") and getattr(getattr(env, "_core", None), "timing_events", None) is None
                and getattr(env, "supports_graph_step", lambda: True)())

    def _train_step_graph(self, device_reset=False):
        eb = self._exp_buffer
        exp_prob = self._get_exp_prob()
        sig = self._env.host_step_signature() if hasattr(self._env, "host_step_signature") else ()
        key = (self._need_normalizer_update(), exp_prob >= 1.0, device_reset) + tuple(sig)
        want = (eb._buffer_head - 1) % eb._buffer_length if self._device_tick() else eb._buffer_head
        if self._head_dev != want:
            self._head_t.fill_(want)
            self._head_dev = want
        if self._exp_prob_dev != exp_prob:
            self._exp_prob_t.fill_(exp_prob)
            self._exp_prob_dev = exp_prob
        g = self._graphs.get(key)
        if g is None:
            if self._graph_warm < 2:
                self._graph_warm += 1
                return self._train_step_body(device_reset)
            eb.set_device_head(self._head_t)
            self._in_graph_step = True
            snapshots = getattr(self._env, "_info_snapshots", None)
            if snapshots is not None:
                self._env._info_snapshots = False
            count0 = self._obs_norm._new_count
            host0 = self._env.host_step_state() if hasattr(self._env, "host_step_state") else None
            captured = False
            try:
                torch.cuda.synchronize()
                g = torch.cuda.CUDAGraph()
                with torch.cuda.graph(g, pool=self._graph_pool, capture_error_mode="thread_local"):
                    done = self._train_step_body(device_reset)
                if self._graph_pool is None:
                    self._graph_pool = g.pool()
                captured = True
            except Exception as exc:
                Logger.print("hipGraph capture of the rollout step failed ({}); continuing with eager launches".format(exc))
                self._use_hip_graph = False
            finally:
                eb.set_device_head(None)
                self._in_graph_step = False
                if snapshots is not None:
                    self._env._info_snapshots = snapshots
            self._obs_norm._new_count = count0
            if not captured:
                torch.cuda.synchronize()
                if hasattr(self._env, "restore_host_step_state"):
                    self._env.restore_host_step_state(host0)
                done = self._train_step_body(False)
                self._graph_fallback_reset = True
                return done
            self._graphs[key] = (g, done)
            fresh = True
        else:
            fresh = False
        g, done = self._graphs[key]
        g.replay()
        if self._device_tick():
            self._head_dev = (self._head_dev + 1) % eb._buffer_length
        if not fresh and hasattr(self._env, "host_step_replayed"):
            self._env.host_step_replayed()
        if key[0]:
            self._obs_norm._new_count += self.get_num_envs()
        self._compute_times.append((eb._buffer_head, time.time() - self._env._start_compute_time))
        return done

    def _flush_compute_times(self):
        if self._compute_times:
            rows = torch.tensor([r for r, _ in self._compute_times], dtype=torch.long, device=self._device)
            vals = torch.tensor([v for _, v in self._compute_times], dtype=torch.float32, device=self._device)
            buf = self._exp_buffer.get_data("compute_time")
            buf[rows] = vals.unsqueeze(1).expand(-1, buf.shape[1])
            self._compute_times = []

    def _rollout_train(self, num_steps):
        for _ in range(num_steps):
            if self._graph_ok():
                dev_reset = self._device_reset_ok()
                done = self._train_step_graph(dev_reset)
                if getattr(self, "_graph_fallback_reset", False):
                    self._graph_fallback_reset = False
                    dev_reset = False
            else:
                dev_reset = False
                done = self._train_step_body()
            if not dev_reset:
                self._curr_obs, self._curr_info = self._reset_done_envs(done)
            self._exp_buffer.inc()
        self._flush_compute_times()

    def _rollout_test(self, num_episodes):
        self._test_return_tracker.reset()
        report_te = getattr(self._env, "_report_tracking_error", False)
        if report_te:
            self._test_tracking_error_tracker.reset()
        if num_episodes == 0:
            return {"mean_return": 0.0, "mean_ep_len": 0.0, "num_eps": 0}
        min_eps_per_env = int(np.ceil(num_episodes / self.get_num_envs()))
        while True:
            action, _ = self._decide_action(self._curr_obs, self._curr_info)
            _, _, done, next_info = self._env.step(action)
            self._test_return_tracker.update(next_info, done)
            if report_te and "tracking_error" in next_info:
                self._test_tracking_error_tracker.update(next_info["tracking_error"], done)
            self._curr_obs, self._curr_info = self._reset_done_envs(done)
            if torch.all(self._test_return_tracker.get_eps_per_env() > min_eps_per_env - 1):
                break
        out = {"mean_return": self._test_return_tracker.get_mean_return().item(),
               "mean_ep_len": self._test_return_tracker.get_mean_ep_len().item(),
               "num_eps": self._test_return_tracker.get_episodes()}
        if report_te:
            t = self._test_tracking_error_tracker
            out.update({"test_mean_root_pos_tracking_err": t.get_mean_root_pos_err().item(),
                        "test_mean_root_rot_tracking_err": t.get_mean_root_rot_err().item(),
                        "test_mean_body_pos_tracking_err": t.get_mean_body_pos_err().item(),
                        "test_mean_body_rot_tracking_err": t.get_mean_body_rot_err().item(),
                        "test_mean_dof_vel_tracking_err": t.get_mean_dof_vel_err().item(),
                        "test_mean_root_vel_tracking_err": t.get_mean_root_vel_err().item(),
                        "test_mean_root_ang_vel_tracking_err": t.get_mean_root_ang_vel_err().item()})
        return out

    def hard_reset_envs(self):
        if self._is_terrain_runner:
            self._env.apply_hard_reset()
        self._curr_obs, self._curr_info = self._env.reset()

    def test_model(self, num_episodes):
        self.eval()
        self.set_mode(AgentMode.TEST)
        self.hard_reset_envs()
        P = mp_util.get_num_procs()
        return self._rollout_test(int(np.ceil(num_episodes / P)))

    @torch.no_grad()
    def _critic_values(self):
        eb = self._exp_buffer
        obs, next_obs, done = eb.get_data("obs"), eb.get_data("next_obs"), eb.get_data("done")
        norm_obs = self._obs_norm.normalize(obs, out=eb.get_data("norm_obs"))
        vals = self._model.eval_critic(norm_obs).squeeze(-1)
        T = obs.shape[0]
        need = done != base_env.DoneFlags.NULL.value
        need[T - 1] = True
        next_vals = torch.empty_like(vals)
        next_vals[:T - 1] = vals[1:]
        idx = need.flatten().nonzero().flatten()
        sel = next_obs.flatten(0, 1)[idx]
        next_vals.flatten()[idx] = self._model.eval_critic(self._obs_norm.normalize(sel)).squeeze(-1)
        return vals, next_vals

    @torch.no_grad()
    def _build_train_data(self):
        self.eval()
        eb = self._exp_buffer
        obs, next_obs = eb.get_data("obs"), eb.get_data("next_obs")
        r, done = eb.get_data("reward"), eb.get_data("done")
        mask = eb.get_data("rand_action_mask")
        vals, next_vals = self._critic_values()
        r_min, r_max = self._env.get_reward_bounds()
        next_vals = torch.clamp(next_vals, r_min / (1.0 - self._discount), r_max / (1.0 - self._discount))
        succ_val = self._env.get_reward_succ() / (1.0 - self._discount)
        fail_val = self._env.get_reward_fail() / (1.0 - self._discount)
        next_vals = torch.where(done == base_env.DoneFlags.SUCC.value, torch.full_like(next_vals, succ_val), next_vals)
        next_vals = torch.where(done == base_env.DoneFlags.FAIL.value, torch.full_like(next_vals, fail_val), next_vals)
        new_vals = rl_util.compute_td_lambda_return(r, next_vals, done, self._discount, self._td_lambda)
        norm_adv, mean_std = rl_util.normalize_advantage(new_vals, vals, mask, self._norm_adv_clip)
        eb.set_data("tar_val", new_vals)
        eb.set_data("adv", norm_adv)
        if eb.has_buffer("loss_rec"):
            rec = eb.get_data("loss_rec")
            A = eb.get_data("action").shape[-1]
            self._a_norm.normalize(eb.get_data("action"), out=rec[..., 0:A])
            rec[..., A] = eb.get_data("a_logp")
            rec[..., A + 1] = norm_adv
            rec[..., A + 2] = mask
            rec[..., A + 3] = new_vals
        return {"adv_mean": mean_std[0], "adv_std": mean_std[1]}

    def _compute_loss(self, batch):
        norm_obs = batch["norm_obs"] if "norm_obs" in batch else self._obs_norm.normalize(batch["obs"])
        norm_a = self._a_norm.normalize(batch["action"])
        pred = self._model.eval_critic(norm_obs).squeeze(-1)
        if norm_obs.is_cuda and self._config.get("fused_ppo_loss", True):
            fused = self._compute_loss_fused(batch, norm_obs, norm_a, pred)
            if fused is not None:
                return fused
        diff = batch["tar_val"] - pred
        critic_loss = torch.mean(torch.square(diff)) if self._critic_loss_type == "L2" else torch.mean(torch.abs(diff))
        m = (batch["rand_action_mask"] == 1.0).to(torch.float32)
        cnt = m.sum().clamp_min(1.0)
        a_dist = self._model.eval_actor(norm_obs)
        a_logp = a_dist.log_prob(norm_a)
        ratio = torch.exp(a_logp - batch["a_logp"])
        adv = batch["adv"]
        l0 = adv * ratio
        l1 = adv * torch.clamp(ratio, 1.0 - self._ppo_clip_ratio, 1.0 + self._ppo_clip_ratio)
        actor_loss = -(torch.minimum(l0, l1) * m).sum() / cnt
        info = {"critic_loss": critic_loss.detach(), "clip_frac": (((torch.abs(ratio - 1.0) > self._ppo_clip_ratio).float() * m).sum() / cnt).detach(),
                "imp_ratio": ((ratio * m).sum() / cnt).detach()}
        if self._action_bound_weight != 0:
            vmin = torch.clamp_max(a_dist.mode + 1.0, 0.0)
            vmax = torch.clamp_min(a_dist.mode - 1.0, 0.0)
            viol = torch.sum(torch.square(vmin), dim=-1) + torch.sum(torch.square(vmax), dim=-1)
            abl = (viol * m).sum() / cnt
            actor_loss = actor_loss + self._action_bound_weight * abl
            info["action_bound_loss"] = abl.detach()
        if self._action_entropy_weight != 0:
            ent = (a_dist.entropy() * m).sum() / cnt
            actor_loss = actor_loss - self._action_entropy_weight * ent
            info["action_entropy"] = ent.detach()
        if self._action_reg_weight != 0:
            reg = (a_dist.param_reg() * m).sum() / cnt
            actor_loss = actor_loss + self._action_reg_weight * reg
            info["action_reg_loss"] = reg.detach()
        info["actor_loss"] = actor_loss.detach()
        actor_term = torch.where(critic_loss.detach() > 20.0, actor_loss.detach(), actor_loss)
        loss = actor_term + self._critic_loss_weight * critic_loss
        info["loss"] = loss
        return info

    def _compute_loss_fused(self, batch, norm_obs, norm_a, pred):
        a_dist = self._model.eval_actor(norm_obs)
        logstd = a_dist.logstd
        if logstd.dim() != 2 or logstd.stride(0) != 0:
            return None
        loss, out = rl_util.ppo_loss(a_dist.mean, logstd[0], pred, norm_a, batch["a_logp"], batch["adv"], batch["rand_action_mask"],
                                     batch["tar_val"], self._ppo_clip_ratio, self._action_bound_weight, self._action_entropy_weight,
                                     self._action_reg_weight, self._critic_loss_weight, 20.0, self._critic_loss_type != "L2")
        slots = {"loss": 0, "critic_loss": 1, "actor_loss": 2, "clip_frac": 3, "imp_ratio": 4}
        if self._action_bound_weight != 0:
            slots["action_bound_loss"] = 5
        if self._action_entropy_weight != 0:
            slots["action_entropy"] = 6
        if self._action_reg_weight != 0:
            slots["action_reg_loss"] = 7
        return {"loss": loss, "_packed": out, "_slots": slots}

    def _explicit_update_ok(self):
        return (str(self._device).startswith("cuda") and self._config.get("explicit_backward", True) and self._config.get("fused_ppo_loss", True)
                and self._model.supports_explicit_backward())

    def _minibatch_step_explicit(self, batch, acc):
        norm_obs = batch["norm_obs"]
        mean, logstd, pred, saved = self._model.train_forward(norm_obs)
        if self._ppo_cfg is None:
            self._ppo_cfg = rl_util.ppo_cfg(self._ppo_clip_ratio, self._action_bound_weight, self._action_entropy_weight, self._action_reg_weight,
                                            self._critic_loss_weight, 20.0, self._critic_loss_type != "L2")
        if "loss_rec" in batch:
            out, g_mean, g_logstd, g_pred = rl_util.ppo_loss_and_grads_packed(mean, logstd, pred, batch["loss_rec"], self._ppo_cfg)
        else:
            out, g_mean, g_logstd, g_pred = rl_util.ppo_loss_and_grads(mean, logstd, pred, self._a_norm.normalize(batch["action"]), batch["a_logp"],
                                                                        batch["adv"], batch["rand_action_mask"], batch["tar_val"], self._ppo_cfg)
        write = lambda grad_of, done: self._model.train_backward(saved, g_mean, g_logstd, g_pred, grad_of, done)
        if self._clip_grad_norm:
            self._optimizer.step_explicit(write, model=self._model, max_norm=self._max_grad_norm)
        else:
            self._optimizer.step_explicit(write)
        acc.append(out)

    def _nan_trap(self, loss_rows, batches, epoch):
        bad = torch.isnan(loss_rows).any(dim=1).tolist()
        if not any(bad):
            return
        k = bad.index(True)
        import pickle
        batch_file = os.path.join("output", "debug_batch.pkl")
        os.makedirs("output", exist_ok=True)
        with open(batch_file, "wb") as f:
            pickle.dump({name: v.detach().cpu() for name, v in batches[k].items()}, f)
        Logger.print("NAN LOSS in minibatch {} of update epoch {}: wrote debug batch file to {}".format(k, epoch, batch_file))
        raise FloatingPointError("NaN loss in minibatch {} of update epoch {} (batch dumped to {}; the reference prints, dumps and exits "
                                 "at this point)".format(k, epoch, batch_file))

    def _update_model(self):
        self.train()
        N = self.get_num_envs()
        num_samples = self._exp_buffer.get_sample_count()
        batch_size = self._batch_size * N
        num_batches = int(np.ceil(float(num_samples) / batch_size))
        acc = dict()
        if self._explicit_update_ok():
            slots = {"loss": 0, "critic_loss": 1, "actor_loss": 2, "clip_frac": 3, "imp_ratio": 4}
            for name, w, i in (("action_bound_loss", self._action_bound_weight, 5), ("action_entropy", self._action_entropy_weight, 6),
                               ("action_reg_loss", self._action_reg_weight, 7)):
                if w != 0:
                    slots[name] = i
            keys = ["norm_obs", "loss_rec"] if self._exp_buffer.has_buffer("loss_rec") else _LOSS_KEYS
            total = None
            for epoch in range(self._update_epochs):
                outs, batches = [], []
                for _ in range(num_batches):
                    batches.append(self._exp_buffer.sample(batch_size, keys=keys))
                    self._minibatch_step_explicit(batches[-1], outs)
                stack = torch.stack(outs)
                self._nan_trap(stack[:, 0:3], batches, epoch)
                total = stack.sum(dim=0) if total is None else total + stack.sum(dim=0)
                del batches
                self._optimizer.end_epoch()
            packed = total / (self._update_epochs * num_batches)
            return {k: packed[i] for k, i in slots.items()}
        for epoch in range(self._update_epochs):
            losses, batches = [], []
            for _ in range(num_batches):
                batch = self._exp_buffer.sample(batch_size, keys=_LOSS_KEYS)
                info = self._compute_loss(batch)
                losses.append(info["loss"].detach())
                batches.append(batch)
                if self._clip_grad_norm:
                    self._optimizer.step(info["loss"], model=self._model, max_norm=self._max_grad_norm)
                else:
                    self._optimizer.step(info["loss"])
                if "_packed" in info:
                    slots = info["_slots"]
                    v = info["_packed"].detach()
                    acc["_packed"] = acc["_packed"] + v if "_packed" in acc else v.clone()
                else:
                    for k, v in info.items():
                        v = v.detach()
                        acc[k] = acc[k] + v if k in acc else v.clone()
            self._nan_trap(torch.stack(losses).reshape(-1, 1), batches, epoch)
            del batches
            self._optimizer.end_epoch()
        steps = self._update_epochs * num_batches
        if "_packed" in acc:
            packed = acc.pop("_packed") / steps
            return {k: packed[i] for k, i in slots.items()}
        return {k: v / steps for k, v in acc.items()}

    def _train_iter(self):
        self._exp_buffer.reset()
        self.eval()
        self.set_mode(AgentMode.TRAIN)
        self._rollout_train(self._steps_per_iter)
        data_info = self._build_train_data()
        train_info = self._update_model()
        if self._need_normalizer_update():
            self._obs_norm.update()
        info = {**train_info, **data_info}
        tr = self._train_return_tracker
        info.update(tr.summary())
        return info

    def _init_train(self):
        self._iter = 0
        self._sample_count = 0
        self._exp_buffer.clear()
        self._train_return_tracker.reset()
        self._test_return_tracker.reset()

    def _update_sample_count(self):
        return mp_util.reduce_sum(self._exp_buffer.get_total_samples())

    def _build_logger(self, log_file):
        log = Logger()
        log.set_step_key("Samples")
        if mp_util.is_root_proc():
            log.configure_output_file(log_file)
        return log

    def _log_train_info(self, train_info, test_info, start_time):
        L = self._logger
        L.log("Iteration", self._iter, collection="1_Info")
        L.log("Wall_Time", (time.time() - start_time) / 3600.0, collection="1_Info")
        L.log("Samples", self._sample_count, collection="1_Info")
        L.log("Test_Return", test_info["mean_return"], collection="0_Main")
        L.log("Test_Episode_Length", test_info["mean_ep_len"], collection="0_Main", quiet=True)
        L.log("Test_Episodes", mp_util.reduce_sum(test_info["num_eps"]), collection="1_Info", quiet=True)
        L.log("Train_Return", train_info.pop("mean_return"), collection="0_Main")
        L.log("Train_Episode_Length", train_info.pop("mean_ep_len"), collection="0_Main", quiet=True)
        L.log("Train_Episodes", mp_util.reduce_sum(train_info.pop("num_eps")), collection="1_Info", quiet=True)
        for k, v in train_info.items():
            if k == "loss":
                v = v.detach()
            L.log(k.title(), v)
        L.log("Exp_Prob", self._get_exp_prob())
        if self._is_terrain_runner:
            L.log("replan timer", self._env.get_replan_time_buf().item())
        if self._log_unit_stats and self._unit_report is not None:
            for l, y in enumerate(self._unit_report["layers"]):
                L.log("Dormant_Pct_L{}".format(l), y["percent_dormant"], collection="3_Units", quiet=True)
                L.log("Act_Mean_L{}".format(l), y["activation"]["mean"], collection="3_Units", quiet=True)
                L.log("Util_Mean_L{}".format(l), y["utility"]["mean"], collection="3_Units", quiet=True)
            L.log("Dormant_Pct_MeanNet", self._unit_report["mean_net"]["percent_dormant"], collection="3_Units", quiet=True)

    def _output_train_model(self, it, out_model_file, int_output_dir):
        self.save(out_model_file)
        if int_output_dir != "":
            self.save(os.path.join(int_output_dir, "model_{:010d}.pt".format(it)))
            if mp_util.is_root_proc() and self._env.has_dm_envs():
                torch.save(self._env.get_dm_env()._motion_id_fail_rates, os.path.join(int_output_dir, "fail_rates_{:010d}.pt".format(it)))

    def train_model(self, max_samples, out_model_file, int_output_dir, log_file, logger_type=None):
        start_time = time.time()
        self._curr_obs, self._curr_info = self._env.reset()
        self._logger = self._build_logger(log_file)
        self._init_train()
        test_info = {"mean_return": 0.0, "mean_ep_len": 0.0, "num_eps": 0}
        while self._sample_count < max_samples:
            train_info = self._train_iter()
            output_iter = (self._iter % self._iters_per_output == 0)
            if output_iter:
                if self._log_unit_stats:
                    self._unit_stats_on()
                try:
                    test_info = self.test_model(self._test_episodes)
                    self._unit_stats_off()
                finally:
                    self._unit_stats = None
                extra = self._env.get_extra_log_info()
                for coll in extra:
                    for k, v in extra[coll].items():
                        self._logger.log(k, v, collection=coll, quiet=True)
                self._env.post_test_update()
            self._sample_count = self._update_sample_count()
            self._log_train_info(train_info, test_info, start_time)
            self._logger.print_log()
            if output_iter:
                self._logger.write_log()
                self._train_return_tracker.reset()
                self.hard_reset_envs()
            if self._iter % self._iters_per_checkpoint == 0:
                self._output_train_model(self._iter, out_model_file, int_output_dir)
            self._iter += 1

    def record_motions(self, max_steps=None):
        self.eval()
        self.set_mode(AgentMode.TEST)
        env = self._env
        env.set_rand_reset(False)
        env.set_demo_mode(True)
        env.set_rand_root_pos_offset_scale(0.0)
        env._episode_length = 1000.0
        N = self.get_num_envs()

        def helper(prev_successful=None):
            self._curr_obs, self._curr_info = env.reset()
            env.build_agent_states_dict("_dm", record_obs=True)
            env.write_agent_states()
            if prev_successful is not None:
                for e in range(N):
                    env.set_writing_env_state(e, not prev_successful[e])
            steps = 0
            while env.is_writing_agent_states() and (max_steps is None or steps < max_steps):
                action, _ = self._decide_action(self._curr_obs, self._curr_info)
                _, _, done, _ = self._env.step(action)
                self._curr_obs, self._curr_info = self._reset_done_envs(done)
                steps += 1

        helper()
        successful = list(env.get_env_success_states())
        counts = [sum(successful)]
        dm = env.get_dm_env()
        clip_len = dm._motion_lib._motion_lengths.cpu().numpy()
        M = dm._motion_lib.num_motions()
        for frac in [0.1, 0.2, 0.3, 0.4, 0.5]:
            if all(successful):
                break
            for e in range(N):
                if (1.0 - frac) * float(clip_len[e % M]) < 2.0:
                    successful[e] = True
            dm.set_motion_start_time_fraction(torch.full([N], frac, dtype=torch.float32, device=self._device))
            helper(prev_successful=successful)
            new = list(env.get_env_success_states())
            counts.append(sum(new))
            successful = [a or b for a, b in zip(successful, new)]
        Logger.print("Successful motions at 0 percent start time: {} / {}".format(counts[0], N))
        Logger.print("Total successful motions: {}".format(sum(counts)))
        return successful


BaseAgent = PPOAgent = DMPPOAgent
```

parc_amd/learning/dm_ppo_model.py:

```python
import enum

import numpy as np
import torch


class StdType(enum.Enum):
    FIXED = 0
    CONSTANT = 1
    VARIABLE = 2


class DistributionGaussianDiag:
    def __init__(self, mean, logstd):
        self._mean = mean
        self._logstd = logstd
        self._std_cache = None
        self._dim = mean.shape[-1]

    @property
    def _std(self):
        if self._std_cache is None:
            self._std_cache = torch.exp(self._logstd)
        return self._std_cache

    @property
    def stddev(self):
        return self._std

    @property
    def logstd(self):
        return self._logstd

    @property
    def mean(self):
        return self._mean

    @property
    def mode(self):
        return self._mean

    def sample(self):
        return self._mean + self._std * torch.randn_like(self._mean)

    def log_prob(self, x):
        diff = x - self._mean
        logp = -0.5 * torch.sum(torch.square(diff / self._std), dim=-1)
        return logp + (-0.5 * self._dim * np.log(2.0 * np.pi) - torch.sum(self._logstd, dim=-1))

    def entropy(self):
        return torch.sum(self._logstd, dim=-1) + 0.5 * self._dim * np.log(2.0 * np.pi * np.e)

    def param_reg(self):
        return torch.sum(torch.square(self._mean), dim=-1)


class DistributionGaussianDiagBuilder(torch.nn.Module):
    def __init__(self, in_size, out_size, std_type, init_std, init_output_scale=0.01):
        super().__init__()
        self._std_type = std_type
        self._mean_net = torch.nn.Linear(in_size, out_size)
        torch.nn.init.uniform_(self._mean_net.weight, -init_output_scale, init_output_scale)
        torch.nn.init.zeros_(self._mean_net.bias)
        logstd = float(np.log(init_std))
        if std_type == StdType.FIXED:
            self._logstd_net = torch.nn.Parameter(torch.full((out_size,), logstd, dtype=torch.float32), requires_grad=False)
        elif std_type == StdType.CONSTANT:
            self._logstd_net = torch.nn.Parameter(torch.full((out_size,), logstd, dtype=torch.float32), requires_grad=True)
        else:
            self._logstd_net = torch.nn.Linear(in_size, out_size)
            torch.nn.init.uniform_(self._logstd_net.weight, -init_output_scale, init_output_scale)
            torch.nn.init.constant_(self._logstd_net.bias, logstd)

    def forward(self, x):
        mean = self._mean_net(x)
        if self._std_type == StdType.VARIABLE:
            logstd = self._logstd_net(x)
        else:
            logstd = torch.broadcast_to(self._logstd_net, mean.shape)
        return DistributionGaussianDiag(mean=mean, logstd=logstd)


_NETS = {"fc_3layers_2048units": [2048, 1024, 512], "fc_3layers_1024units": [1024, 1024, 512], "fc_2layers_1024units": [1024, 512]}


class _LinearReLU(torch.autograd.Function):

    @staticmethod
    def forward(ctx, x, weight, bias):
        y = torch._addmm_activation(bias, x, weight.t(), use_gelu=False)
        ctx.save_for_backward(x, weight, y)
        return y

    @staticmethod
    def backward(ctx, gy):
        x, weight, y = ctx.saved_tensors
        g = torch.ops.aten.threshold_backward(gy, y, 0.0)
        gx = g.mm(weight) if ctx.needs_input_grad[0] else None
        gw = g.t().mm(x) if ctx.needs_input_grad[1] else None
        gb = g.sum(dim=0) if ctx.needs_input_grad[2] else None
        return gx, gw, gb


class FusedMLP(torch.nn.Sequential):

    def forward(self, x):
        mods = list(self)
        if not (x.is_cuda and x.dim() == 2 and x.dtype == torch.float32):
            return super().forward(x)
        i = 0
        while i < len(mods):
            m = mods[i]
            if isinstance(m, torch.nn.Linear) and i + 1 < len(mods) and isinstance(mods[i + 1], torch.nn.ReLU):
                if torch.is_grad_enabled() and (x.requires_grad or m.weight.requires_grad):
                    x = _LinearReLU.apply(x, m.weight, m.bias)
                else:
                    x = torch._addmm_activation(m.bias, x, m.weight.t(), use_gelu=False)
                i += 2
            else:
                x = m(x)
                i += 1
        return x


def build_net(name, in_size, activation):
    if name not in _NETS:
        raise NotImplementedError("net '{}' (the tracker default is fc_3layers_2048units)".format(name))
    layers = []
    for out_size in _NETS[name]:
        lin = torch.nn.Linear(in_size, out_size)
        torch.nn.init.zeros_(lin.bias)
        layers += [lin, activation()]
        in_size = out_size
    return FusedMLP(*layers), in_size


class DMPPOModel(torch.nn.Module):
    def __init__(self, config, env):
        super().__init__()
        self._activation = torch.nn.ReLU
        obs_dim = int(np.prod(env.get_obs_space().shape))
        a_dim = int(np.prod(env.get_action_space().shape))
        self._actor_layers, h = build_net(config["actor_net"], obs_dim, self._activation)
        self._action_dist = DistributionGaussianDiagBuilder(h, a_dim, std_type=StdType[config["actor_std_type"]],
                                                            init_std=config["action_std"],
                                                            init_output_scale=config["actor_init_output_scale"])
        self._critic_layers, hc = build_net(config["critic_net"], obs_dim, self._activation)
        self._critic_out = torch.nn.Linear(hc, 1)
        torch.nn.init.zeros_(self._critic_out.bias)

    def eval_actor(self, obs):
        return self._action_dist(self._actor_layers(obs))

    @torch.no_grad()
    def eval_actor_tapped(self, obs):
        acts = self._trunk_forward(self._actor_layers, obs)
        mnet = self._action_dist._mean_net
        mean = torch.addmm(mnet.bias, acts[-1], mnet.weight.t())
        return DistributionGaussianDiag(mean=mean, logstd=torch.broadcast_to(self._action_dist._logstd_net, mean.shape)), acts[1:]

    def supports_explicit_backward(self):
        def plain(seq):
            mods = list(seq)
            return len(mods) % 2 == 0 and all(isinstance(m, torch.nn.Linear) for m in mods[0::2]) and all(isinstance(m, torch.nn.ReLU) for m in mods[1::2]) \
                and all(m.out_features % 4 == 0 for m in mods[0::2])
        return plain(self._actor_layers) and plain(self._critic_layers) and self._action_dist._std_type != StdType.VARIABLE

    @staticmethod
    def _trunk_forward(seq, x):
        acts = [x]
        for lin in list(seq)[0::2]:
            x = torch._addmm_activation(lin.bias, x, lin.weight.t(), use_gelu=False)
            acts.append(x)
        return acts

    @torch.no_grad()
    def train_forward(self, norm_obs):
        a = self._trunk_forward(self._actor_layers, norm_obs)
        c = self._trunk_forward(self._critic_layers, norm_obs)
        mnet = self._action_dist._mean_net
        mean = torch.addmm(mnet.bias, a[-1], mnet.weight.t())
        pred = torch.addmm(self._critic_out.bias, c[-1], self._critic_out.weight.t()).squeeze(-1)
        return mean, self._action_dist._logstd_net, pred, (a, c)

    def _relu_bwd(self, d, y, db):
        from .. import _hip
        L = _hip.lib()
        need = int(L.parc_relu_bwd_workspace_floats(d.shape[0], d.shape[1]))
        ws = getattr(self, "_relu_ws", None)
        if ws is None or ws.numel() < need or ws.device != d.device:
            ws = self._relu_ws = torch.empty(max(need, 1), dtype=torch.float32, device=d.device)
        _hip.check(L.parc_relu_bwd_bias_grad(_hip.stream(), d.shape[0], d.shape[1], _hip.ptr(d), _hip.ptr(y), _hip.ptr(db), _hip.ptr(ws)),
                   "parc_relu_bwd_bias_grad")

    def _weighted_colsum(self, x, w, out):
        from .. import _hip
        L = _hip.lib()
        need = int(L.parc_relu_bwd_workspace_floats(x.shape[0], x.shape[1]))
        ws = getattr(self, "_relu_ws", None)
        if ws is None or ws.numel() < need or ws.device != x.device:
            ws = self._relu_ws = torch.empty(max(need, 1), dtype=torch.float32, device=x.device)
        _hip.check(L.parc_weighted_colsum(_hip.stream(), x.shape[0], x.shape[1], _hip.ptr(x), _hip.ptr(w.contiguous()), _hip.ptr(out), _hip.ptr(ws)),
                   "parc_weighted_colsum")

    def _trunk_backward(self, seq, acts, d, grad_of, done):
        lins = list(seq)[0::2]
        for k in range(len(lins) - 1, -1, -1):
            lin = lins[k]
            self._relu_bwd(d, acts[k + 1], grad_of(lin.bias))
            torch.mm(d.t(), acts[k], out=grad_of(lin.weight))
            done(lin.weight)
            done(lin.bias)
            if k > 0:
                d = torch.mm(d, lin.weight)

    @torch.no_grad()
    def train_backward(self, saved, g_mean, g_logstd, g_pred, grad_of, done=lambda p: None):
        a, c = saved
        mnet = self._action_dist._mean_net
        torch.mm(g_mean.t(), a[-1], out=grad_of(mnet.weight))
        torch.sum(g_mean, dim=0, out=grad_of(mnet.bias))
        done(mnet.weight)
        done(mnet.bias)
        if self._action_dist._std_type == StdType.CONSTANT:
            grad_of(self._action_dist._logstd_net).copy_(g_logstd)
            done(self._action_dist._logstd_net)
        self._trunk_backward(self._actor_layers, a, torch.mm(g_mean, mnet.weight), grad_of, done)
        gp = g_pred.unsqueeze(-1)
        if self._critic_out.weight.shape[0] == 1:
            self._weighted_colsum(c[-1], g_pred, grad_of(self._critic_out.weight).view(-1))
        else:
            torch.mm(gp.t(), c[-1], out=grad_of(self._critic_out.weight))
        torch.sum(gp, dim=0, out=grad_of(self._critic_out.bias))
        done(self._critic_out.weight)
        done(self._critic_out.bias)
        self._trunk_backward(self._critic_layers, c, torch.mm(gp, self._critic_out.weight), grad_of, done)

    def eval_critic(self, obs):
        return self._critic_out(self._critic_layers(obs))
```

Before: 453,900 env-steps/s.

## Fuse PPO policy/value heads with loss and head backward into custom kernels

Adds a kernel that computes the actor mean and critic value heads together with the packed PPO loss and its gradients. It also adds a head backward kernel that fuses the head weight/bias gradients, the trunk-input gradient and the last ReLU bias gradient, applying the loss scale inside. The aim is to drop several small GEMM, reduction and elementwise launches per minibatch and avoid materialising mean/pred and scaled gradients. Fallbacks to the old path remain for unsupported shapes, at the cost of more code and possible numeric-ordering differences.

```diff
diff --git a/include/parc_hip.h b/include/parc_hip.h
--- a/include/parc_hip.h
+++ b/include/parc_hip.h
@@ -246,6 +246,13 @@
 int parc_relu_bwd_bias_grad(void *stream, int64_t rows, int dim, float *gy, const float *y, float *db, float *workspace);
 int parc_weighted_colsum(void *stream, int64_t rows, int dim, const float *x, const float *w, float *out, float *workspace);
 
+int parc_ppo_heads_forward(void *stream, int B, int A, int H, const float *a3, const float *c3, const float *Wm, const float *bm, const float *wc,
+                           const float *bc, const float *logstd, const float *rec, int rec_stride, parc_ppo_cfg_t cfg, float *mean, float *pred,
+                           float *g_mean, float *g_logstd, float *g_pred, float *out, float *workspace);
+int64_t parc_head_backward_workspace_floats(int64_t rows, int dim, int A);
+int parc_head_backward(void *stream, int64_t rows, int dim, int A, const float *y, const float *g, const float *scale, const float *W, float *d,
+                       float *db_trunk, float *dW_head, float *db_head, float *workspace);
+
 int parc_abi_version(void);
 
 #ifdef __cplusplus
diff --git a/parc_amd/_hip.py b/parc_amd/_hip.py
--- a/parc_amd/_hip.py
+++ b/parc_amd/_hip.py
@@ -8,7 +8,7 @@
 LIB_DIR = os.path.join(_HERE, "lib")
 LIB_PATH = os.path.join(LIB_DIR, "libparc_hip.so")
 CSRC = os.path.join(_HERE, "csrc")
-SOURCES = ["parc_kin.hip", "parc_sim.hip", "parc_ppo.hip", "parc_rollout.hip", "parc_optim.hip", "parc_colreduce.hip", "parc_terrain.hip", "parc_render.hip", "parc_score.hip", "parc_netstats.hip", "parc_moopt.hip",
+SOURCES = ["parc_kin.hip", "parc_sim.hip", "parc_ppo.hip", "parc_rollout.hip", "parc_optim.hip", "parc_colreduce.hip", "parc_ppo_heads.hip", "parc_terrain.hip", "parc_render.hip", "parc_score.hip", "parc_netstats.hip", "parc_moopt.hip",
            "parc_augment.hip", "parc_mdm_batch.hip", "parc_mdm_loss.hip", "parc_mdm_guide.hip", "parc_mdm_gen.hip", "parc_hfgather.hip", "parc_motion.hip", "parc_pose_opt.hip", "parc_returns.hip"]
 DIAG_LIB_PATH = os.path.join(LIB_DIR, "libparc_hip_diag.so")
 DIAG_SOURCES = SOURCES + ["parc_sim_ref.hip"]
@@ -229,6 +229,12 @@
     L.parc_relu_bwd_bias_grad.restype = c_int
     L.parc_weighted_colsum.argtypes = [c_vp, c_i64, c_int, c_vp, c_vp, c_vp, c_vp]
     L.parc_weighted_colsum.restype = c_int
+    L.parc_ppo_heads_forward.argtypes = [c_vp, c_int, c_int, c_int] + [c_vp] * 8 + [c_int, PPOCfgS] + [c_vp] * 7
+    L.parc_ppo_heads_forward.restype = c_int
+    L.parc_head_backward_workspace_floats.argtypes = [c_i64, c_int, c_int]
+    L.parc_head_backward_workspace_floats.restype = c_i64
+    L.parc_head_backward.argtypes = [c_vp, c_i64, c_int, c_int] + [c_vp] * 9
+    L.parc_head_backward.restype = c_int
     L.parc_sgd_workspace_floats.argtypes = []
     L.parc_sgd_workspace_floats.restype = c_i64
     L.parc_sgd_momentum_step.argtypes = [c_vp, c_i64, c_vp, c_vp, c_vp, c_f, c_f, c_f, c_f, c_vp, c_vp]
@@ -289,7 +295,7 @@
             "parc_forward_kinematics", "parc_calc_motion_frame", "parc_motion_lib_build", "parc_track_post_step",
             "parc_update_fail_rates", "parc_td_lambda_return", "parc_adv_normalize", "parc_reset_apply", "parc_ppo_loss", "parc_ppo_workspace_floats", "parc_record_step", "parc_return_tracker_update", "parc_normalize_clamp",
             "parc_action_head", "parc_points_hf_sdf", "parc_moments_workspace_floats", "parc_moments_accumulate", "parc_reset_sample_apply", "parc_return_tracker_workspace_floats", "parc_scale_by_clipped_norm", "parc_relu_bwd_workspace_floats",
-            "parc_relu_bwd_bias_grad", "parc_ppo_loss_packed", "parc_weighted_colsum", "parc_sgd_workspace_floats", "parc_sgd_momentum_step", "parc_adamw_step",
+            "parc_relu_bwd_bias_grad", "parc_ppo_loss_packed", "parc_weighted_colsum", "parc_ppo_heads_forward", "parc_head_backward_workspace_floats", "parc_head_backward", "parc_sgd_workspace_floats", "parc_sgd_momentum_step", "parc_adamw_step",
             "parc_pose_chain_forward", "parc_pose_chain_backward", "parc_points_hf_sdf_grad", "parc_body_points_world", "parc_body_points_world_grad",
             "parc_quat_diff_angle", "parc_quat_diff_angle_grad", "parc_temporal_terms", "parc_temporal_terms_grad", "parc_step_tail",
             "parc_assemble_obs", "parc_track_post_step_timed", "parc_rng_step", "parc_obs_ingest", "parc_action_head_record",
@@ -304,6 +310,9 @@
             "parc_mdm_gen_encode", "parc_mdm_gen_decode", "parc_mdm_gen_abi"]
 
 
+EUNSUPPORTED = -2
+
+
 def check(rc, what):
     if rc != 0:
         raise RuntimeError("{} failed with code {} ({})".format(what, rc, "bad argument" if rc == -1 else "unsupported" if rc == -2 else "hipError"))
diff --git a/parc_amd/csrc/parc_col_chunk.h b/parc_amd/csrc/parc_col_chunk.h
--- /dev/null
+++ b/parc_amd/csrc/parc_col_chunk.h
@@ -0,0 +1,49 @@
+#pragma once
+#include <hip/hip_runtime.h>
+#include <stdint.h>
+
+#include "../../include/parc_hip.h"
+
+#define RB_ROWS 128
+
+struct col_chunk_t {
+    int lane, rg, c, r0, r1;
+};
+
+__device__ __forceinline__ col_chunk_t col_chunk(int rows, int chunk_rows) {
+    const int lane = threadIdx.x & 63, r0 = blockIdx.y * chunk_rows;
+    return {lane, (int)(threadIdx.x >> 6), (int)(blockIdx.x * 64 + lane), r0, min(r0 + chunk_rows, rows)};
+}
+
+__device__ __forceinline__ float4 fold_row_groups(const float4 (*red)[64], int lane) {
+    const float4 a = red[0][lane], b = red[1][lane], d = red[2][lane], e = red[3][lane];
+    float4 o;
+    o.x = (a.x + b.x) + (d.x + e.x); o.y = (a.y + b.y) + (d.y + e.y); o.z = (a.z + b.z) + (d.z + e.z); o.w = (a.w + b.w) + (d.w + e.w);
+    return o;
+}
+
+__device__ __forceinline__ void fold_store(float4 (*red)[64], const float4 &s, const col_chunk_t &k, int dim4, float4 *__restrict__ partial) {
+    red[k.rg][k.lane] = s;
+    __syncthreads();
+    if (k.rg == 0 && k.c < dim4) partial[(size_t)blockIdx.y * dim4 + k.c] = fold_row_groups(red, k.lane);
+}
+
+__device__ __forceinline__ void fold_store_moments(float4 (*red)[4][64], const float4 &s, const float4 &q, const col_chunk_t &k, int dim4,
+                                                   float4 *__restrict__ partial) {
+    red[0][k.rg][k.lane] = s;
+    red[1][k.rg][k.lane] = q;
+    __syncthreads();
+    if (k.rg < 2 && k.c < dim4) partial[((size_t)blockIdx.y * 2 + k.rg) * dim4 + k.c] = fold_row_groups(red[k.rg], k.lane);
+}
+
+struct col_grid_t {
+    int rc, dim4, chunks;
+    dim3 grid;
+};
+
+static inline col_grid_t col_chunk_grid(int64_t rows, int dim, int chunk_rows, uintptr_t aligned16, bool missing) {
+    if (rows < 0 || dim <= 0 || (dim & 3) || missing || (aligned16 & 15)) return {PARC_EINVAL};
+    if (rows > (int64_t)chunk_rows * 65535) return {PARC_EUNSUPPORTED};
+    const int dim4 = dim / 4, chunks = (int)((rows + chunk_rows - 1) / chunk_rows);
+    return {PARC_OK, dim4, chunks, dim3((dim4 + 63) / 64, chunks)};
+}
diff --git a/parc_amd/csrc/parc_colreduce.hip b/parc_amd/csrc/parc_colreduce.hip
--- a/parc_amd/csrc/parc_colreduce.hip
+++ b/parc_amd/csrc/parc_colreduce.hip
@@ -2,6 +2,7 @@
 #include <stdint.h>
 
 #include "../../include/parc_hip.h"
+#include "parc_col_chunk.h"
 #include "parc_launch.h"
 #include "parc_learner_math.h"
 
@@ -28,48 +29,6 @@
                        (const float4 *)mean, (const float4 *)stdv, clip, (float4 *)out);
     PARC_CHECK_LAUNCH();
     return PARC_OK;
-}
-
-struct col_chunk_t {
-    int lane, rg, c, r0, r1;
-};
-
-__device__ __forceinline__ col_chunk_t col_chunk(int rows, int chunk_rows) {
-    const int lane = threadIdx.x & 63, r0 = blockIdx.y * chunk_rows;
-    return {lane, (int)(threadIdx.x >> 6), (int)(blockIdx.x * 64 + lane), r0, min(r0 + chunk_rows, rows)};
-}
-
-__device__ __forceinline__ float4 fold_row_groups(const float4 (*red)[64], int lane) {
-    const float4 a = red[0][lane], b = red[1][lane], d = red[2][lane], e = red[3][lane];
-    float4 o;
-    o.x = (a.x + b.x) + (d.x + e.x); o.y = (a.y + b.y) + (d.y + e.y); o.z = (a.z + b.z) + (d.z + e.z); o.w = (a.w + b.w) + (d.w + e.w);
-    return o;
-}
-
-__device__ __forceinline__ void fold_store(float4 (*red)[64], const float4 &s, const col_chunk_t &k, int dim4, float4 *__restrict__ partial) {
-    red[k.rg][k.lane] = s;
-    __syncthreads();
-    if (k.rg == 0 && k.c < dim4) partial[(size_t)blockIdx.y * dim4 + k.c] = fold_row_groups(red, k.lane);
-}
-
-__device__ __forceinline__ void fold_store_moments(float4 (*red)[4][64], const float4 &s, const float4 &q, const col_chunk_t &k, int dim4,
-                                                   float4 *__restrict__ partial) {
-    red[0][k.rg][k.lane] = s;
-    red[1][k.rg][k.lane] = q;
-    __syncthreads();
-    if (k.rg < 2 && k.c < dim4) partial[((size_t)blockIdx.y * 2 + k.rg) * dim4 + k.c] = fold_row_groups(red[k.rg], k.lane);
-}
-
-struct col_grid_t {
-    int rc, dim4, chunks;
-    dim3 grid;
-};
-
-static col_grid_t col_chunk_grid(int64_t rows, int dim, int chunk_rows, uintptr_t aligned16, bool missing) {
-    if (rows < 0 || dim <= 0 || (dim & 3) || missing || (aligned16 & 15)) return {PARC_EINVAL};
-    if (rows > (int64_t)chunk_rows * 65535) return {PARC_EUNSUPPORTED};
-    const int dim4 = dim / 4, chunks = (int)((rows + chunk_rows - 1) / chunk_rows);
-    return {PARC_OK, dim4, chunks, dim3((dim4 + 63) / 64, chunks)};
 }
 
 #define MOM_ROWS 64
@@ -167,7 +126,6 @@
     return PARC_OK;
 }
 
-#define RB_ROWS 128
 __global__ __launch_bounds__(256) void relu_bwd_bias_partial_kernel(int rows, int dim4, float4 *__restrict__ gy, const float4 *__restrict__ y,
                                                                     float4 *__restrict__ partial) {
     __shared__ float4 red[4][64];
diff --git a/parc_amd/csrc/parc_ppo.hip b/parc_amd/csrc/parc_ppo.hip
--- a/parc_amd/csrc/parc_ppo.hip
+++ b/parc_amd/csrc/parc_ppo.hip
@@ -3,34 +3,9 @@
 #include "../../include/parc_hip.h"
 #include "parc_launch.h"
 #include "parc_learner_math.h"
+#include "parc_ppo_sample.h"
 
 #define PPO_THREADS 256
-#define PPO_MAX_A 64
-#define PPO_NSCAL 8
-#define PPO_W (PPO_NSCAL + PPO_MAX_A)
-
-struct ppo_surr_t {
-    float ratio, surr, c;
-};
-
-__device__ __forceinline__ ppo_surr_t ppo_surrogate(int A, float zz, float sum_logstd, const float *old_logp, const float *adv, size_t si, bool sel,
-                                                    float m, parc_ppo_cfg_t cfg) {
-    ppo_surr_t s;
-    const float logp = -0.5f * zz + (-0.5f * (float)A * 1.8378770664093453f - sum_logstd);
-    s.ratio = __expf(logp - old_logp[si]);
-    const float ad = adv[si];
-    const float lo = 1.0f - cfg.clip_ratio, hi = 1.0f + cfg.clip_ratio;
-    const float rc = clamp_nan(s.ratio, lo, hi);
-    const float l0 = ad * s.ratio, l1 = ad * rc;
-    s.surr = minimum_nan(l0, l1);
-    const float dsurr = (l0 <= l1) ? ad : ((s.ratio >= lo && s.ratio <= hi) ? ad : 0.f);
-    s.c = sel ? -m * dsurr * s.ratio : 0.f;
-    return s;
-}
-
-__device__ __forceinline__ float ppo_critic_grad(parc_ppo_cfg_t cfg, float diff) {
-    return cfg.critic_l1 ? (diff > 0.f ? -1.f : (diff < 0.f ? 1.f : 0.f)) : -2.0f * diff;
-}
 
 __global__ __launch_bounds__(PPO_THREADS) void ppo_sample_kernel(int B, int A, const float *__restrict__ mean, const float *__restrict__ logstd,
                                                                  const float *__restrict__ norm_a, const float *__restrict__ old_logp,
@@ -102,7 +77,6 @@
     }
 }
 
-#define PPO32_SPB 64
 __global__ __launch_bounds__(256) void ppo_sample32_kernel(int B, int A, const float *__restrict__ mean, const float *__restrict__ logstd,
                                                            const float *__restrict__ norm_a, const float *__restrict__ old_logp,
                                                            const float *__restrict__ adv, const float *__restrict__ mask,
@@ -110,63 +84,17 @@
                                                            float *g_mean, float *g_pred, float *ws, int a_stride, int s_stride) {
     __shared__ float s_part[8][PPO_W];
     const int tid = threadIdx.x, g = tid >> 5, j = tid & 31;
-    const bool vj = j < A;
-    const float ls = vj ? logstd[j] : 0.f;
-    const float istd = __expf(-ls);
-    float sum_logstd = ls;
-#pragma unroll
-    for (int o = 16; o >= 1; o >>= 1) sum_logstd += __shfl_xor(sum_logstd, o, 32);
-    float acc[PPO_NSCAL];
-#pragma unroll
-    for (int k = 0; k < PPO_NSCAL; ++k) acc[k] = 0.f;
-    float acc_ls = 0.f;
+    const ppo32_lane_t l = ppo32_lane(A, j, logstd);
+    ppo32_acc_t acc = ppo32_acc_zero();
 #pragma unroll 2
     for (int it = 0; it < PPO32_SPB / 8; ++it) {
         const int i = blockIdx.x * PPO32_SPB + it * 8 + g;
         const bool live = i < B;
         const int ii = live ? i : 0;
-        const size_t si = (size_t)ii * s_stride;
-        const bool sel = live && mask[si] == 1.0f;
-        const float m = sel ? 1.f : 0.f;
-        const float mj = vj ? mean[(size_t)ii * A + j] : 0.f;
-        const float aj = vj ? norm_a[(size_t)ii * a_stride + j] : 0.f;
-        const float z = (aj - mj) * istd;
-        const float vmin = clamp_max_nan(mj + 1.0f, 0.f), vmax = clamp_min_nan(mj - 1.0f, 0.f);
-        float zz = vj ? z * z : 0.f, viol = vj ? vmin * vmin + vmax * vmax : 0.f, reg = vj ? mj * mj : 0.f;
-#pragma unroll
-        for (int o = 16; o >= 1; o >>= 1) {
-            zz += __shfl_xor(zz, o, 32);
-            viol += __shfl_xor(viol, o, 32);
-            reg += __shfl_xor(reg, o, 32);
-        }
-        const ppo_surr_t sr = ppo_surrogate(A, zz, sum_logstd, old_logp, adv, si, sel, m, cfg);
-        const float c = sr.c;
-        const float diff = tar_val[si] - pred[ii];
-        if (live) {
-            if (j == 0) g_pred[i] = ppo_critic_grad(cfg, diff);
-            if (vj) g_mean[(size_t)i * A + j] = sel ? c * z * istd + m * (cfg.bound_w * 2.0f * (vmin + vmax) + cfg.reg_w * 2.0f * mj) : 0.f;
-        }
-        acc[0] += m;
-        acc[1] += live ? (cfg.critic_l1 ? fabsf(diff) : diff * diff) : 0.f;
-        acc[2] += sel ? m * sr.surr : 0.f;
-        acc[3] += m * (fabsf(sr.ratio - 1.0f) > cfg.clip_ratio ? 1.f : 0.f);
-        acc[4] += sel ? m * sr.ratio : 0.f;
-        acc[5] += sel ? m * viol : 0.f;
-        acc[6] += sel ? m * reg : 0.f;
-        acc_ls += (sel && vj) ? c * (z * z - 1.0f) : 0.f;
+        const float mj = l.vj ? mean[(size_t)ii * A + j] : 0.f;
+        ppo32_sample(acc, A, i, ii, live, j, l, mj, pred[ii], norm_a, old_logp, adv, mask, tar_val, cfg, g_mean, g_pred, a_stride, s_stride);
     }
-    if (j == 0) {
-#pragma unroll
-        for (int k = 0; k < PPO_NSCAL; ++k) s_part[g][k] = acc[k];
-    }
-    if (vj) s_part[g][PPO_NSCAL + j] = acc_ls;
-    __syncthreads();
-    if (tid < PPO_NSCAL + A) {
-        float v = 0.f;
-#pragma unroll
-        for (int w = 0; w < 8; ++w) v += s_part[w][tid];
-        ws[(size_t)blockIdx.x * PPO_W + tid] = v;
-    }
+    ppo32_store_partial(acc, A, g, j, l.vj, s_part, ws);
 }
 
 #define PPO_RED_THREADS (4 * PPO_W)
@@ -216,6 +144,10 @@
     }
 }
 
+void ppo_launch_reduce(void *stream, int B, int A, int nblk, const float *logstd, parc_ppo_cfg_t cfg, const float *ws, float *g_logstd, float *out) {
+    hipLaunchKernelGGL(ppo_reduce_kernel, dim3(1), dim3(PPO_RED_THREADS), 0, (hipStream_t)stream, B, A, nblk, logstd, cfg, ws, g_logstd, out);
+}
+
 __global__ __launch_bounds__(256) void ppo_scale_kernel(int n_mean, int n_pred, const float *__restrict__ out, float *g_mean, float *g_pred) {
     const int i = blockIdx.x * blockDim.x + threadIdx.x;
     const float sa = out[9], sp = out[10];
@@ -237,7 +169,7 @@
         hipLaunchKernelGGL(ppo_sample_kernel, dim3(nblk), dim3(PPO_THREADS), 0, st, B, A, mean, logstd, norm_a, old_logp, adv, mask, pred, tar_val,
                            cfg, g_mean, g_pred, workspace, a_stride, s_stride);
     }
-    hipLaunchKernelGGL(ppo_reduce_kernel, dim3(1), dim3(PPO_RED_THREADS), 0, st, B, A, nblk, logstd, cfg, workspace, g_logstd, out);
+    ppo_launch_reduce(stream, B, A, nblk, logstd, cfg, workspace, g_logstd, out);
     const int n = B * A;
     hipLaunchKernelGGL(ppo_scale_kernel, dim3((n + 255) / 256), dim3(256), 0, st, n, B, out, g_mean, g_pred);
     PARC_CHECK_LAUNCH();
diff --git a/parc_amd/csrc/parc_ppo_heads.hip b/parc_amd/csrc/parc_ppo_heads.hip
--- /dev/null
+++ b/parc_amd/csrc/parc_ppo_heads.hip
@@ -0,0 +1,256 @@
+#include <hip/hip_runtime.h>
+#include <stdint.h>
+
+#include "../../include/parc_hip.h"
+#include "parc_col_chunk.h"
+#include "parc_launch.h"
+#include "parc_learner_math.h"
+#include "parc_ppo_sample.h"
+
+__device__ __forceinline__ float4 ld4_or_zero(bool ok, const float4 *__restrict__ p) {
+    float4 v = make_float4(0.f, 0.f, 0.f, 0.f);
+    if (ok) v = *p;
+    return v;
+}
+
+#define HF_KC4 32
+#define HF_LD4 (HF_KC4 + 1)
+
+__global__ __launch_bounds__(256) void ppo_heads_forward_kernel(int B, int A, int H4, const float4 *__restrict__ a3, const float4 *__restrict__ c3,
+                                                                const float4 *__restrict__ Wm, const float *__restrict__ bm,
+                                                                const float4 *__restrict__ wc, const float *__restrict__ bc,
+                                                                const float *__restrict__ logstd, const float *__restrict__ rec, int rec_stride,
+                                                                parc_ppo_cfg_t cfg, float *mean_out, float *pred_out, float *g_mean, float *g_pred,
+                                                                float *ws) {
+    __shared__ float4 sA[PPO32_SPB][HF_LD4];
+    __shared__ float4 sW[32][HF_LD4];
+    __shared__ float s_part[8][PPO_W];
+    const int tid = threadIdx.x, g = tid >> 5, j = tid & 31;
+    const int row0 = blockIdx.x * PPO32_SPB;
+
+    float pr[PPO32_SPB / 8];
+#pragma unroll
+    for (int it = 0; it < PPO32_SPB / 8; ++it) pr[it] = 0.f;
+    for (int q = j; q < H4; q += 32) {
+        const float4 w = wc[q];
+#pragma unroll
+        for (int it = 0; it < PPO32_SPB / 8; ++it) {
+            const int i = row0 + it * 8 + g;
+            const float4 v = c3[(size_t)(i < B ? i : 0) * H4 + q];
+            pr[it] = fmaf(v.x, w.x, pr[it]); pr[it] = fmaf(v.y, w.y, pr[it]); pr[it] = fmaf(v.z, w.z, pr[it]); pr[it] = fmaf(v.w, w.w, pr[it]);
+        }
+    }
+    const float bcv = bc[0];
+#pragma unroll
+    for (int it = 0; it < PPO32_SPB / 8; ++it) {
+#pragma unroll
+        for (int o = 16; o >= 1; o >>= 1) pr[it] += __shfl_xor(pr[it], o, 32);
+        pr[it] += bcv;
+    }
+
+    float mu[PPO32_SPB / 8];
+#pragma unroll
+    for (int it = 0; it < PPO32_SPB / 8; ++it) mu[it] = 0.f;
+    float4 ra[PPO32_SPB * HF_KC4 / 256], rw[32 * HF_KC4 / 256];
+    const int sr = tid >> 5, sq = tid & 31;
+#define HF_LOAD(k0)                                                                                                              \
+    do {                                                                                                                         \
+        const bool cv = (k0) + sq < H4;                                                                                          \
+        _Pragma("unroll") for (int t = 0; t < PPO32_SPB / 8; ++t) {                                                              \
+            const int r = row0 + t * 8 + sr;                                                                                     \
+            ra[t] = ld4_or_zero(cv && r < B, a3 + ((size_t)r * H4 + (k0) + sq));                                                 \
+        }                                                                                                                        \
+        _Pragma("unroll") for (int t = 0; t < 4; ++t) {                                                                          \
+            const int a = t * 8 + sr;                                                                                            \
+            rw[t] = ld4_or_zero(cv && a < A, Wm + ((size_t)a * H4 + (k0) + sq));                                                 \
+        }                                                                                                                        \
+    } while (0)
+    HF_LOAD(0);
+    for (int k0 = 0; k0 < H4; k0 += HF_KC4) {
+        if (k0) __syncthreads();
+#pragma unroll
+        for (int t = 0; t < PPO32_SPB / 8; ++t) sA[t * 8 + sr][sq] = ra[t];
+#pragma unroll
+        for (int t = 0; t < 4; ++t) sW[t * 8 + sr][sq] = rw[t];
+        __syncthreads();
+        if (k0 + HF_KC4 < H4) HF_LOAD(k0 + HF_KC4);
+        const int nq = min(HF_KC4, H4 - k0);
+        for (int q = 0; q < nq; ++q) {
+            const float4 w = sW[j][q];
+#pragma unroll
+            for (int it = 0; it < PPO32_SPB / 8; ++it) {
+                const float4 v = sA[it * 8 + g][q];
+                mu[it] = fmaf(v.x, w.x, mu[it]); mu[it] = fmaf(v.y, w.y, mu[it]); mu[it] = fmaf(v.z, w.z, mu[it]); mu[it] = fmaf(v.w, w.w, mu[it]);
+            }
+        }
+    }
+#undef HF_LOAD
+
+    const ppo32_lane_t l = ppo32_lane(A, j, logstd);
+    const float bmj = l.vj ? bm[j] : 0.f;
+    ppo32_acc_t acc = ppo32_acc_zero();
+#pragma unroll
+    for (int it = 0; it < PPO32_SPB / 8; ++it) {
+        const int i = row0 + it * 8 + g;
+        const bool live = i < B;
+        const int ii = live ? i : 0;
+        const float mj = l.vj ? mu[it] + bmj : 0.f;
+        if (live) {
+            if (mean_out && l.vj) mean_out[(size_t)i * A + j] = mj;
+            if (pred_out && j == 0) pred_out[i] = pr[it];
+        }
+        ppo32_sample(acc, A, i, ii, live, j, l, mj, pr[it], rec, rec + A, rec + A + 1, rec + A + 2, rec + A + 3, cfg, g_mean, g_pred, rec_stride,
+                     rec_stride);
+    }
+    ppo32_store_partial(acc, A, g, j, l.vj, s_part, ws);
+}
+
+extern "C" int parc_ppo_heads_forward(void *stream, int B, int A, int H, const float *a3, const float *c3, const float *Wm, const float *bm,
+                                      const float *wc, const float *bc, const float *logstd, const float *rec, int rec_stride, parc_ppo_cfg_t cfg,
+                                      float *mean, float *pred, float *g_mean, float *g_logstd, float *g_pred, float *out, float *workspace) {
+    if (B <= 0 || A <= 0 || H <= 0 || !a3 || !c3 || !Wm || !bm || !wc || !bc || !logstd || !rec || rec_stride < A + 4 || !g_mean || !g_logstd ||
+        !g_pred || !out || !workspace)
+        return PARC_EINVAL;
+    if (A > 32 || (H & 3) || (((uintptr_t)a3 | (uintptr_t)c3 | (uintptr_t)Wm | (uintptr_t)wc) & 15)) return PARC_EUNSUPPORTED;
+    const int nblk = (B + PPO32_SPB - 1) / PPO32_SPB;
+    hipLaunchKernelGGL(ppo_heads_forward_kernel, dim3(nblk), dim3(256), 0, (hipStream_t)stream, B, A, H / 4, (const float4 *)a3, (const float4 *)c3,
+                       (const float4 *)Wm, bm, (const float4 *)wc, bc, logstd, rec, rec_stride, cfg, mean, pred, g_mean, g_pred, workspace);
+    ppo_launch_reduce(stream, B, A, nblk, logstd, cfg, workspace, g_logstd, out);
+    PARC_CHECK_LAUNCH();
+    return PARC_OK;
+}
+
+template <int AT>
+__global__ __launch_bounds__(256) void head_backward_partial_kernel(int rows, int dim4, int A, const float4 *__restrict__ y, const float *__restrict__ g,
+                                                                    const float *__restrict__ scale, const float4 *__restrict__ W,
+                                                                    float4 *__restrict__ d, float4 *__restrict__ p_db, float4 *__restrict__ p_dW,
+                                                                    float *__restrict__ p_dbh) {
+    constexpr int RT = AT >= 4 ? AT / 4 : 1;
+    constexpr int NR = AT / RT;
+    __shared__ float4 sW[AT >= 4 ? AT : 4][64];
+    __shared__ __attribute__((aligned(16))) float sg[RB_ROWS][AT];
+    __shared__ float4 red[4][64];
+    __shared__ float s_bh[4][32];
+    const col_chunk_t k = col_chunk(rows, RB_ROWS);
+    const int tid = threadIdx.x, lane = k.lane, rg = k.rg, c = k.c, r0 = k.r0, r1 = k.r1;
+    const float4 zero4 = make_float4(0.f, 0.f, 0.f, 0.f);
+    const float s = scale[0];
+    for (int idx = tid; idx < (r1 - r0) * AT; idx += 256) {
+        const int r = idx / AT, a = idx - r * AT;
+        sg[r][a] = a < A ? g[(size_t)(r0 + r) * A + a] * s : 0.f;
+    }
+    for (int idx = tid; idx < AT * 64; idx += 256) {
+        const int a = idx >> 6, cc = blockIdx.x * 64 + (idx & 63);
+        sW[a][idx & 63] = ld4_or_zero(a < A && cc < dim4, W + ((size_t)a * dim4 + cc));
+    }
+    __syncthreads();
+    if (blockIdx.x == 0 && lane < AT) {
+        float t = 0.f;
+        for (int r = rg; r < r1 - r0; r += 4) t += sg[r][lane];
+        s_bh[rg][lane & 31] = t;
+    }
+    float4 sdb = zero4, dW[AT];
+#pragma unroll
+    for (int a = 0; a < AT; ++a) dW[a] = zero4;
+    if (c < dim4) {
+#pragma unroll 2
+        for (int r = r0 + rg; r < r1; r += 4) {
+            const size_t i = (size_t)r * dim4 + c;
+            const float4 v = y[i];
+            float sv[AT];
+            if constexpr (AT >= 4) {
+#pragma unroll
+                for (int a4 = 0; a4 < AT / 4; ++a4) {
+                    const float4 t = *reinterpret_cast<const float4 *>(&sg[r - r0][a4 * 4]);
+                    sv[a4 * 4] = t.x; sv[a4 * 4 + 1] = t.y; sv[a4 * 4 + 2] = t.z; sv[a4 * 4 + 3] = t.w;
+                }
+            } else {
+#pragma unroll
+                for (int a = 0; a < AT; ++a) sv[a] = sg[r - r0][a];
+            }
+            float4 dv;
+            {
+                const float4 w = sW[0][lane];
+                dv.x = sv[0] * w.x; dv.y = sv[0] * w.y; dv.z = sv[0] * w.z; dv.w = sv[0] * w.w;
+            }
+#pragma unroll
+            for (int a = 1; a < AT; ++a) {
+                const float4 w = sW[a][lane];
+                dv.x = fmaf(sv[a], w.x, dv.x); dv.y = fmaf(sv[a], w.y, dv.y); dv.z = fmaf(sv[a], w.z, dv.z); dv.w = fmaf(sv[a], w.w, dv.w);
+            }
+#pragma unroll
+            for (int a = 0; a < AT; ++a) {
+                dW[a].x = fmaf(sv[a], v.x, dW[a].x); dW[a].y = fmaf(sv[a], v.y, dW[a].y); dW[a].z = fmaf(sv[a], v.z, dW[a].z);
+                dW[a].w = fmaf(sv[a], v.w, dW[a].w);
+            }
+            dv.x = v.x <= 0.f ? 0.f : dv.x; dv.y = v.y <= 0.f ? 0.f : dv.y; dv.z = v.z <= 0.f ? 0.f : dv.z; dv.w = v.w <= 0.f ? 0.f : dv.w;
+            d[i] = dv;
+            sdb.x += dv.x; sdb.y += dv.y; sdb.z += dv.z; sdb.w += dv.w;
+        }
+    }
+    fold_store(red, sdb, k, dim4, p_db);
+    if (blockIdx.x == 0 && tid < A) p_dbh[(size_t)blockIdx.y * A + tid] = (s_bh[0][tid] + s_bh[1][tid]) + (s_bh[2][tid] + s_bh[3][tid]);
+    float4 (*park)[4][64] = reinterpret_cast<float4 (*)[4][64]>(&sW[0][0]);
+#pragma unroll
+    for (int q = 0; q < NR; ++q) {
+        if (q) __syncthreads();
+#pragma unroll
+        for (int t = 0; t < RT; ++t) park[t][rg][lane] = dW[q * RT + t];
+        __syncthreads();
+        for (int t = rg; t < RT; t += 4) {
+            const int a = q * RT + t;
+            if (a < A && c < dim4) p_dW[((size_t)blockIdx.y * A + a) * dim4 + c] = fold_row_groups(park[t], lane);
+        }
+    }
+}
+
+__global__ __launch_bounds__(256) void head_backward_fold_kernel(int chunks, int A, int dim, const float *__restrict__ p_db, const float *__restrict__ p_dW,
+                                                                 const float *__restrict__ p_dbh, float *__restrict__ db_trunk,
+                                                                 float *__restrict__ dW_head, float *__restrict__ db_head) {
+    const int i = blockIdx.x * blockDim.x + threadIdx.x;
+    const int n_w = A * dim;
+    const float *src;
+    float *dst;
+    int stride;
+    if (i < dim) {
+        src = p_db + i; dst = db_trunk + i; stride = dim;
+    } else if (i < dim + n_w) {
+        src = p_dW + (i - dim); dst = dW_head + (i - dim); stride = n_w;
+    } else if (i < dim + n_w + A) {
+        src = p_dbh + (i - dim - n_w); dst = db_head + (i - dim - n_w); stride = A;
+    } else {
+        return;
+    }
+    float t = 0.f;
+#pragma unroll 16
+    for (int kk = 0; kk < chunks; ++kk) t += src[(size_t)kk * stride];
+    *dst = t;
+}
+
+extern "C" int64_t parc_head_backward_workspace_floats(int64_t rows, int dim, int A) {
+    if (rows < 0 || dim <= 0 || A <= 0) return -1;
+    return ((rows + RB_ROWS - 1) / RB_ROWS) * ((int64_t)dim * (A + 1) + A);
+}
+
+extern "C" int parc_head_backward(void *stream, int64_t rows, int dim, int A, const float *y, const float *g, const float *scale, const float *W,
+                                  float *d, float *db_trunk, float *dW_head, float *db_head, float *workspace) {
+    if (rows < 0 || dim <= 0 || A <= 0 || !y || !g || !scale || !W || !d || !db_trunk || !dW_head || !db_head || !workspace) return PARC_EINVAL;
+    if (A > 32 || (dim & 3) || (((uintptr_t)y | (uintptr_t)W | (uintptr_t)d | (uintptr_t)workspace) & 15)) return PARC_EUNSUPPORTED;
+    const col_grid_t cg = col_chunk_grid(rows, dim, RB_ROWS, 0, false);
+    if (cg.rc != PARC_OK) return cg.rc;
+    float *p_db = workspace, *p_dW = p_db + (size_t)cg.chunks * dim, *p_dbh = p_dW + (size_t)cg.chunks * A * dim;
+    if (rows > 0) {
+#define HB_LAUNCH(AT)                                                                                                                        \
+    hipLaunchKernelGGL(head_backward_partial_kernel<AT>, cg.grid, dim3(256), 0, (hipStream_t)stream, (int)rows, cg.dim4, A, (const float4 *)y, g, \
+                       scale, (const float4 *)W, (float4 *)d, (float4 *)p_db, (float4 *)p_dW, p_dbh)
+        if (A == 1) HB_LAUNCH(1);
+        else if (A == 28) HB_LAUNCH(28);
+        else HB_LAUNCH(32);
+#undef HB_LAUNCH
+    }
+    const int n = dim * (A + 1) + A;
+    hipLaunchKernelGGL(head_backward_fold_kernel, dim3((n + 255) / 256), dim3(256), 0, (hipStream_t)stream, cg.chunks, A, dim, p_db, p_dW, p_dbh,
+                       db_trunk, dW_head, db_head);
+    PARC_CHECK_LAUNCH();
+    return PARC_OK;
+}
diff --git a/parc_amd/csrc/parc_ppo_sample.h b/parc_amd/csrc/parc_ppo_sample.h
--- /dev/null
+++ b/parc_amd/csrc/parc_ppo_sample.h
@@ -0,0 +1,116 @@
+#pragma once
+#include <hip/hip_runtime.h>
+
+#include "../../include/parc_hip.h"
+#include "parc_learner_math.h"
+
+#define PPO_MAX_A 64
+#define PPO_NSCAL 8
+#define PPO_W (PPO_NSCAL + PPO_MAX_A)
+#define PPO32_SPB 64
+
+__attribute__((visibility("hidden"))) void ppo_launch_reduce(void *stream, int B, int A, int nblk, const float *logstd, parc_ppo_cfg_t cfg,
+                                                             const float *ws, float *g_logstd, float *out);
+
+struct ppo_surr_t {
+    float ratio, surr, c;
+};
+
+__device__ __forceinline__ ppo_surr_t ppo_surrogate(int A, float zz, float sum_logstd, const float *old_logp, const float *adv, size_t si, bool sel,
+                                                    float m, parc_ppo_cfg_t cfg) {
+    ppo_surr_t s;
+    const float logp = -0.5f * zz + (-0.5f * (float)A * 1.8378770664093453f - sum_logstd);
+    s.ratio = __expf(logp - old_logp[si]);
+    const float ad = adv[si];
+    const float lo = 1.0f - cfg.clip_ratio, hi = 1.0f + cfg.clip_ratio;
+    const float rc = clamp_nan(s.ratio, lo, hi);
+    const float l0 = ad * s.ratio, l1 = ad * rc;
+    s.surr = minimum_nan(l0, l1);
+    const float dsurr = (l0 <= l1) ? ad : ((s.ratio >= lo && s.ratio <= hi) ? ad : 0.f);
+    s.c = sel ? -m * dsurr * s.ratio : 0.f;
+    return s;
+}
+
+__device__ __forceinline__ float ppo_critic_grad(parc_ppo_cfg_t cfg, float diff) {
+    return cfg.critic_l1 ? (diff > 0.f ? -1.f : (diff < 0.f ? 1.f : 0.f)) : -2.0f * diff;
+}
+
+struct ppo32_lane_t {
+    bool vj;
+    float istd, sum_logstd;
+};
+
+__device__ __forceinline__ ppo32_lane_t ppo32_lane(int A, int j, const float *__restrict__ logstd) {
+    ppo32_lane_t l;
+    l.vj = j < A;
+    const float ls = l.vj ? logstd[j] : 0.f;
+    l.istd = __expf(-ls);
+    l.sum_logstd = ls;
+#pragma unroll
+    for (int o = 16; o >= 1; o >>= 1) l.sum_logstd += __shfl_xor(l.sum_logstd, o, 32);
+    return l;
+}
+
+struct ppo32_acc_t {
+    float s[PPO_NSCAL], ls;
+};
+
+__device__ __forceinline__ ppo32_acc_t ppo32_acc_zero() {
+    ppo32_acc_t a;
+#pragma unroll
+    for (int k = 0; k < PPO_NSCAL; ++k) a.s[k] = 0.f;
+    a.ls = 0.f;
+    return a;
+}
+
+__device__ __forceinline__ void ppo32_sample(ppo32_acc_t &acc, int A, int i, int ii, bool live, int j, const ppo32_lane_t &l, float mj, float pred_i,
+                                             const float *__restrict__ norm_a, const float *__restrict__ old_logp, const float *__restrict__ adv,
+                                             const float *__restrict__ mask, const float *__restrict__ tar_val, parc_ppo_cfg_t cfg, float *g_mean,
+                                             float *g_pred, int a_stride, int s_stride) {
+    const bool vj = l.vj;
+    const float istd = l.istd;
+    const size_t si = (size_t)ii * s_stride;
+    const bool sel = live && mask[si] == 1.0f;
+    const float m = sel ? 1.f : 0.f;
+    const float aj = vj ? norm_a[(size_t)ii * a_stride + j] : 0.f;
+    const float z = (aj - mj) * istd;
+    const float vmin = clamp_max_nan(mj + 1.0f, 0.f), vmax = clamp_min_nan(mj - 1.0f, 0.f);
+    float zz = vj ? z * z : 0.f, viol = vj ? vmin * vmin + vmax * vmax : 0.f, reg = vj ? mj * mj : 0.f;
+#pragma unroll
+    for (int o = 16; o >= 1; o >>= 1) {
+        zz += __shfl_xor(zz, o, 32);
+        viol += __shfl_xor(viol, o, 32);
+        reg += __shfl_xor(reg, o, 32);
+    }
+    const ppo_surr_t sr = ppo_surrogate(A, zz, l.sum_logstd, old_logp, adv, si, sel, m, cfg);
+    const float c = sr.c;
+    const float diff = tar_val[si] - pred_i;
+    if (live) {
+        if (j == 0) g_pred[i] = ppo_critic_grad(cfg, diff);
+        if (vj) g_mean[(size_t)i * A + j] = sel ? c * z * istd + m * (cfg.bound_w * 2.0f * (vmin + vmax) + cfg.reg_w * 2.0f * mj) : 0.f;
+    }
+    acc.s[0] += m;
+    acc.s[1] += live ? (cfg.critic_l1 ? fabsf(diff) : diff * diff) : 0.f;
+    acc.s[2] += sel ? m * sr.surr : 0.f;
+    acc.s[3] += m * (fabsf(sr.ratio - 1.0f) > cfg.clip_ratio ? 1.f : 0.f);
+    acc.s[4] += sel ? m * sr.ratio : 0.f;
+    acc.s[5] += sel ? m * viol : 0.f;
+    acc.s[6] += sel ? m * reg : 0.f;
+    acc.ls += (sel && vj) ? c * (z * z - 1.0f) : 0.f;
+}
+
+__device__ __forceinline__ void ppo32_store_partial(const ppo32_acc_t &acc, int A, int g, int j, bool vj, float (*s_part)[PPO_W], float *ws) {
+    if (j == 0) {
+#pragma unroll
+        for (int k = 0; k < PPO_NSCAL; ++k) s_part[g][k] = acc.s[k];
+    }
+    if (vj) s_part[g][PPO_NSCAL + j] = acc.ls;
+    __syncthreads();
+    const int tid = threadIdx.x;
+    if (tid < PPO_NSCAL + A) {
+        float v = 0.f;
+#pragma unroll
+        for (int w = 0; w < 8; ++w) v += s_part[w][tid];
+        ws[(size_t)blockIdx.x * PPO_W + tid] = v;
+    }
+}
diff --git a/parc_amd/learning/dm_ppo_agent.py b/parc_amd/learning/dm_ppo_agent.py
--- a/parc_amd/learning/dm_ppo_agent.py
+++ b/parc_amd/learning/dm_ppo_agent.py
@@ -616,16 +616,27 @@
 
     def _minibatch_step_explicit(self, batch, acc):
         norm_obs = batch["norm_obs"]
-        mean, logstd, pred, saved = self._model.train_forward(norm_obs)
         if self._ppo_cfg is None:
             self._ppo_cfg = rl_util.ppo_cfg(self._ppo_clip_ratio, self._action_bound_weight, self._action_entropy_weight, self._action_reg_weight,
                                             self._critic_loss_weight, 20.0, self._critic_loss_type != "L2")
+        fused = None
         if "loss_rec" in batch:
+            _, logstd, _, saved = self._model.train_forward(norm_obs, heads=False)
+            fused = self._model.heads_forward_loss(saved, batch["loss_rec"], self._ppo_cfg)
+            if fused is None:
+                mean, pred = self._model.head_outputs(saved)
+        else:
+            mean, logstd, pred, saved = self._model.train_forward(norm_obs)
+        scale = None
+        if fused is not None:
+            out, g_mean, g_logstd, g_pred = fused
+            scale = out
+        elif "loss_rec" in batch:
             out, g_mean, g_logstd, g_pred = rl_util.ppo_loss_and_grads_packed(mean, logstd, pred, batch["loss_rec"], self._ppo_cfg)
         else:
             out, g_mean, g_logstd, g_pred = rl_util.ppo_loss_and_grads(mean, logstd, pred, self._a_norm.normalize(batch["action"]), batch["a_logp"],
                                                                         batch["adv"], batch["rand_action_mask"], batch["tar_val"], self._ppo_cfg)
-        write = lambda grad_of, done: self._model.train_backward(saved, g_mean, g_logstd, g_pred, grad_of, done)
+        write = lambda grad_of, done: self._model.train_backward(saved, g_mean, g_logstd, g_pred, grad_of, done, scale=scale)
         if self._clip_grad_norm:
             self._optimizer.step_explicit(write, model=self._model, max_norm=self._max_grad_norm)
         else:
diff --git a/parc_amd/learning/dm_ppo_model.py b/parc_amd/learning/dm_ppo_model.py
--- a/parc_amd/learning/dm_ppo_model.py
+++ b/parc_amd/learning/dm_ppo_model.py
@@ -174,13 +174,72 @@
         return acts
 
     @torch.no_grad()
-    def train_forward(self, norm_obs):
+    def train_forward(self, norm_obs, heads=True):
         a = self._trunk_forward(self._actor_layers, norm_obs)
         c = self._trunk_forward(self._critic_layers, norm_obs)
+        mean, pred = self.head_outputs((a, c)) if heads else (None, None)
+        return mean, self._action_dist._logstd_net, pred, (a, c)
+
+    @torch.no_grad()
+    def head_outputs(self, saved):
+        a, c = saved
         mnet = self._action_dist._mean_net
         mean = torch.addmm(mnet.bias, a[-1], mnet.weight.t())
         pred = torch.addmm(self._critic_out.bias, c[-1], self._critic_out.weight.t()).squeeze(-1)
-        return mean, self._action_dist._logstd_net, pred, (a, c)
+        return mean, pred
+
+    def _head_buf(self, key, numel, device):
+        bufs = self.__dict__.setdefault("_head_bufs", dict())
+        t = bufs.get(key)
+        if t is None or t.numel() < numel or t.device != device:
+            t = bufs[key] = torch.empty(max(int(numel), 1), dtype=torch.float32, device=device)
+        return t
+
+    @torch.no_grad()
+    def heads_forward_loss(self, saved, rec, cfg):
+        from .. import _hip
+        a3, c3 = saved[0][-1], saved[1][-1]
+        mnet, cnet = self._action_dist._mean_net, self._critic_out
+        if self._action_dist._std_type == StdType.VARIABLE or cnet.weight.shape[0] != 1 or not a3.is_cuda or a3.shape != c3.shape:
+            return None
+        tensors = (a3, c3, mnet.weight, mnet.bias, cnet.weight, cnet.bias, self._action_dist._logstd_net, rec)
+        if not all(t.dtype == torch.float32 and t.is_contiguous() for t in tensors):
+            return None
+        B, H = a3.shape
+        A = mnet.weight.shape[0]
+        L, p, dev = _hip.lib(), _hip.ptr, a3.device
+        g_mean = torch.empty(B, A, dtype=torch.float32, device=dev)
+        g_logstd = torch.empty(A, dtype=torch.float32, device=dev)
+        g_pred = torch.empty(B, dtype=torch.float32, device=dev)
+        out = torch.empty(16, dtype=torch.float32, device=dev)
+        ws = self._head_buf("loss", L.parc_ppo_workspace_floats(B), dev)
+        rc = L.parc_ppo_heads_forward(_hip.stream(), B, A, H, p(a3), p(c3), p(mnet.weight), p(mnet.bias), p(cnet.weight), p(cnet.bias),
+                                      p(self._action_dist._logstd_net), p(rec), int(rec.shape[1]), cfg, None, None, p(g_mean), p(g_logstd),
+                                      p(g_pred), p(out), p(ws))
+        if rc == _hip.EUNSUPPORTED:
+            return None
+        _hip.check(rc, "parc_ppo_heads_forward")
+        return out, g_mean, g_logstd, g_pred
+
+    def _head_backward(self, key, y, g, scale, head, l3_bias, grad_of):
+        from .. import _hip
+        W = head.weight
+        if not (y.is_cuda and y.is_contiguous() and g.is_contiguous() and W.is_contiguous() and W.dtype == torch.float32):
+            return None
+        L, p = _hip.lib(), _hip.ptr
+        rows, dim = y.shape
+        A = W.shape[0]
+        need = int(L.parc_head_backward_workspace_floats(rows, dim, A))
+        if need < 0:
+            return None
+        ws = self._head_buf("bwd", need, y.device)
+        d = self._head_buf("d_" + key, rows * dim, y.device)[:rows * dim].view(rows, dim)
+        rc = L.parc_head_backward(_hip.stream(), rows, dim, A, p(y), p(g), p(scale), p(W), p(d), p(grad_of(l3_bias)), p(grad_of(W)),
+                                  p(grad_of(head.bias)), p(ws))
+        if rc == _hip.EUNSUPPORTED:
+            return None
+        _hip.check(rc, "parc_head_backward")
+        return d
 
     def _relu_bwd(self, d, y, db):
         from .. import _hip
@@ -202,11 +261,12 @@
         _hip.check(L.parc_weighted_colsum(_hip.stream(), x.shape[0], x.shape[1], _hip.ptr(x), _hip.ptr(w.contiguous()), _hip.ptr(out), _hip.ptr(ws)),
                    "parc_weighted_colsum")
 
-    def _trunk_backward(self, seq, acts, d, grad_of, done):
+    def _trunk_backward(self, seq, acts, d, grad_of, done, last_masked=False):
         lins = list(seq)[0::2]
         for k in range(len(lins) - 1, -1, -1):
             lin = lins[k]
-            self._relu_bwd(d, acts[k + 1], grad_of(lin.bias))
+            if not (last_masked and k == len(lins) - 1):
+                self._relu_bwd(d, acts[k + 1], grad_of(lin.bias))
             torch.mm(d.t(), acts[k], out=grad_of(lin.weight))
             done(lin.weight)
             done(lin.bias)
@@ -214,17 +274,36 @@
                 d = torch.mm(d, lin.weight)
 
     @torch.no_grad()
-    def train_backward(self, saved, g_mean, g_logstd, g_pred, grad_of, done=lambda p: None):
+    def train_backward(self, saved, g_mean, g_logstd, g_pred, grad_of, done=lambda p: None, scale=None):
         a, c = saved
         mnet = self._action_dist._mean_net
-        torch.mm(g_mean.t(), a[-1], out=grad_of(mnet.weight))
-        torch.sum(g_mean, dim=0, out=grad_of(mnet.bias))
+        d = None
+        if scale is not None:
+            d = self._head_backward("actor", a[-1], g_mean, scale[9:10], mnet, list(self._actor_layers)[-2].bias, grad_of)
+            if d is None:
+                g_mean = g_mean * scale[9]
+        if d is None:
+            torch.mm(g_mean.t(), a[-1], out=grad_of(mnet.weight))
+            torch.sum(g_mean, dim=0, out=grad_of(mnet.bias))
         done(mnet.weight)
         done(mnet.bias)
         if self._action_dist._std_type == StdType.CONSTANT:
             grad_of(self._action_dist._logstd_net).copy_(g_logstd)
             done(self._action_dist._logstd_net)
-        self._trunk_backward(self._actor_layers, a, torch.mm(g_mean, mnet.weight), grad_of, done)
+        if d is None:
+            self._trunk_backward(self._actor_layers, a, torch.mm(g_mean, mnet.weight), grad_of, done)
+        else:
+            self._trunk_backward(self._actor_layers, a, d, grad_of, done, last_masked=True)
+        d = None
+        if scale is not None:
+            d = self._head_backward("critic", c[-1], g_pred, scale[10:11], self._critic_out, list(self._critic_layers)[-2].bias, grad_of)
+            if d is None:
+                g_pred = g_pred * scale[10]
+        if d is not None:
+            done(self._critic_out.weight)
+            done(self._critic_out.bias)
+            self._trunk_backward(self._critic_layers, c, d, grad_of, done, last_masked=True)
+            return
         gp = g_pred.unsqueeze(-1)
         if self._critic_out.weight.shape[0] == 1:
             self._weighted_colsum(c[-1], g_pred, grad_of(self._critic_out.weight).view(-1))
```

Measured after the change: 458,100 env-steps/s (median of 6 runs). Within noise of the previous version (+0.9%).
